# tangjiapeng/DiffuScene

Hardware: AMD Instinct MI355X
Metric: denoiser steps/sec (train + 1000-step sample) at B=256, N=80 objects (higher is better)
Workload: dtype f32 (operands split 3xbf16, 6 products, f32 accumulate); 1 GPU; uncond living/dining rooms (config/uncond/diffusion_livingrooms_instancond_lat32_v.yaml scaled to N=80), B=256 scenes per GPU, N=80, C=65, T=1000, mode=both; global_batch=256, parallelism=single

## Files before the change

__graft_entry__.py:

```python
import os
import subprocess
import sys

ROOT = os.path.dirname(os.path.abspath(__file__))
CSRC = os.path.join(ROOT, "diffuscene_amd", "csrc")
LIB = os.path.join(ROOT, "diffuscene_amd", "libdiffuscene_hip.so")

SOURCES = [
    ("gemm_mfma.hip", []),
    ("gemm_split.hip", ["-fno-slp-vectorize"]),
    ("gemm_tn_split.hip", ["-fno-slp-vectorize"]),
    ("blocks.hip", []),
    ("diffusion.hip", ["-ffp-contract=off"]),
    ("train.hip", []),
    ("retrieval.hip", ["-ffp-contract=off"]),
    ("dataset.hip", ["-ffp-contract=off"]),
    ("chamfer.hip", ["-ffp-contract=off"]),
    ("optim.hip", ["-ffp-contract=off"]),
    ("foldingnet.hip", []),
]


def _hipcc():
    for c in (os.environ.get("HIPCC"), "/opt/rocm/bin/hipcc", "hipcc"):
        if c and (os.path.isabs(c) and os.path.exists(c) or not os.path.isabs(c)):
            return c
    raise RuntimeError("hipcc not found")


def _stale(target, deps):
    if not os.path.exists(target):
        return True
    t = os.path.getmtime(target)
    return any(os.path.getmtime(d) > t for d in deps)


def _stamp_git_head():
    try:
        head = subprocess.check_output(["git", "rev-parse", "--short", "HEAD"], cwd=ROOT, stderr=subprocess.DEVNULL, text=True).strip()
        dirty = subprocess.check_output(["git", "status", "--porcelain", "-uno"], cwd=ROOT, stderr=subprocess.DEVNULL, text=True).strip()
        with open(os.path.join(ROOT, "GIT_HEAD"), "w") as f:
            f.write(head + ("+" if dirty else "") + "\n")
    except Exception:
        pass


def build(force=False):
    hipcc = _hipcc()
    headers = [os.path.join(CSRC, "dsc_common.h"), os.path.join(CSRC, "gemm_core.h"), os.path.join(CSRC, "gemm_tn_split.h"),
               os.path.join(ROOT, "include", "diffuscene_hip.h")]
    objs = []
    for src, extra in SOURCES:
        s = os.path.join(CSRC, src)
        if not os.path.exists(s):
            continue
        o = os.path.join(CSRC, src.replace(".hip", ".o"))
        if force or _stale(o, [s] + headers):
            cmd = [hipcc, "--offload-arch=gfx950", "-O3", "-std=c++17", "-fPIC", "-c", s, "-o", o] + extra
            subprocess.check_call(cmd)
        objs.append(o)
    if force or _stale(LIB, objs):
        subprocess.check_call([hipcc, "--offload-arch=gfx950", "-shared", "-fPIC", "-o", LIB] + objs)
    gsrc = os.path.join(ROOT, "tools", "guard_alloc.cpp")
    gso = os.path.join(ROOT, "tools", "_build", "libdsc_guard_alloc.so")
    if os.path.exists(gsrc) and (force or _stale(gso, [gsrc])):
        os.makedirs(os.path.dirname(gso), exist_ok=True)
        try:
            subprocess.check_call([hipcc, "-O2", "-std=c++17", "-fPIC", "-shared", gsrc, "-o", gso])
        except (subprocess.CalledProcessError, OSError) as e:
            print("warning: guard allocator (tools/guard_alloc.cpp) not built: %s -- tests/test_gpu_guard.py will skip its allocator runs" % e,
                  file=sys.stderr)
    _stamp_git_head()
    if ROOT not in sys.path:
        sys.path.insert(0, ROOT)
    import diffuscene_amd
    from diffuscene_amd import _lib
    _lib.load()
    import oracle.ref_torch


def build_asan():
    hipcc = _hipcc()
    out = os.path.join(ROOT, "diffuscene_amd", "libdiffuscene_hip_asan.so")
    objs = []
    for src, extra in SOURCES:
        s = os.path.join(CSRC, src)
        o = os.path.join(CSRC, src.replace(".hip", ".asan.o"))
        subprocess.check_call([hipcc, "--offload-arch=gfx950", "-O1", "-g", "-std=c++17", "-fPIC", "-fsanitize=address", "-fno-gpu-sanitize",
                               "-shared-libsan", "-Wno-option-ignored", "-c", s, "-o", o] + extra)
        objs.append(o)
    subprocess.check_call([hipcc, "--offload-arch=gfx950", "-shared", "-fPIC", "-fsanitize=address", "-fno-gpu-sanitize", "-shared-libsan",
                           "-Wno-option-ignored", "-o", out] + objs)
    return out


def smoke():
    if ROOT not in sys.path:
        sys.path.insert(0, ROOT)
    import torch
    assert torch.cuda.is_available(), "smoke() needs a GPU"
    from diffuscene_amd.networks.denoise_net import Unet1D
    from diffuscene_amd.networks.diffusion_ddpm import DiffusionPoint
    from oracle import ref_torch as R
    from oracle import weights as W

    kw = dict(W.UNCOND_BEDROOM)
    B, N = 4, 12
    dev = torch.device("cuda:0")
    net = Unet1D(**kw)
    sd = W.synth_state_dict(kw)
    net.load_state_dict(sd)
    net.to(dev)
    cfg = dict(objectness_dim=0, class_dim=22, angle_dim=2, objfeat_dim=32)
    diff = DiffusionPoint(net, cfg, time_num=1000, model_mean_type="v")
    x = W.synth_scene_batch(B, N, 22, 32, 0)
    t = torch.tensor([3, 250, 600, 999], dtype=torch.int64)
    cond = W.synth_condition(B, N, 128, 0).contiguous()
    noise = W.synth_noise((B, N, 62), 7)
    with torch.no_grad():
        out = net(x.to(dev), t.to(dev), cond.to(dev), None).cpu()
        ref = R.unet1d_forward(sd, kw, x, t, cond, None)
        rel = float((out - ref).abs().max() / ref.abs().max())
        assert rel < 1e-4, "Unet1D forward mismatch vs oracle: %g" % rel
        tb = R.schedule_tables(1e-4, 0.02, 1000, "v")
        step = diff.diffusion.p_sample(diff._denoise, x.to(dev), t.to(dev), cond.to(dev), None,
                                       noise_fn=lambda size, dtype, device: noise.to(device), clip_denoised=True).cpu()
        ref_step = R.p_sample_step(tb, x, t, ref, noise, True, "v")
        rel2 = float((step - ref_step).abs().max() / ref_step.abs().max())
        assert rel2 < 1e-4, "p_sample mismatch vs oracle: %g" % rel2
    print("smoke ok: forward rel err %.3g, p_sample rel err %.3g" % (rel, rel2))


if __name__ == "__main__":
    if "--asan" in sys.argv:
        print("built", build_asan())
        sys.exit(0)
    build(force="--force" in sys.argv)
    if "--smoke" in sys.argv:
        smoke()
```

diffuscene_amd/_lib.py:

```python
import ctypes as C
import os

_HERE = os.path.dirname(os.path.abspath(__file__))
LIB_PATH = os.path.join(_HERE, "libdiffuscene_hip.so")
if os.environ.get("DSC_HIP_LIB"):
    LIB_PATH = os.path.abspath(os.environ["DSC_HIP_LIB"])

ACT_NONE, ACT_GELU, ACT_SILU, ACT_LEAKY01 = 0, 1, 2, 3
SS_NONE, SS_PER_TOKEN, SS_PER_SCENE, SS_PER_SLOT, SS_BY_INDEX = 0, 1, 2, 3, 4
MEAN_EPS, MEAN_X0, MEAN_V = 0, 1, 2
TILE_GN_80_W8, TILE_GN_80_W4, TILE_160x256, TILE_160x128_W4 = 1, 2, 5, 8
TILE_WAVE_GN, TILE_WAVE_DENSE, TILE_WAVE_GN_64 = 10, 11, 12
F32_TILE_160x256, F32_TILE_160x128, F32_TILE_128x128, F32_TILE_96x128, F32_TILE_64x64 = 0, 1, 2, 3, 4
DSC_PLANES_NONE = -100
GEMM_ROW_INVARIANT = 1
WS_MAX = 64
MAX_TOKENS_PER_SCENE = 160
STATS_MAX_OBJECTS, STATS_ONE_WAVE_MAX = 160, 32

_ERR = {-1: "DSC_EINVAL (bad shape / null pointer)", -2: "DSC_EALIGN (16-byte alignment required)",
        -3: "DSC_ERANGE (size outside kernel limits)"}

c_f32p = C.c_void_p
c_i64p = C.c_void_p


class GemmArgs(C.Structure):
    _fields_ = [
        ("a1", C.c_void_p), ("lda1", C.c_int64), ("k1", C.c_int32),
        ("a2", C.c_void_p), ("lda2", C.c_int64), ("k2", C.c_int32),
        ("w", C.c_void_p), ("ldw", C.c_int64),
        ("bias", C.c_void_p),
        ("residual", C.c_void_p), ("ldr", C.c_int64),
        ("y", C.c_void_p), ("ldy", C.c_int64),
        ("m", C.c_int32), ("n", C.c_int32),
        ("act_in", C.c_int32), ("act_out", C.c_int32),
        ("batch", C.c_int32),
        ("sa1", C.c_int64), ("sa2", C.c_int64), ("sw", C.c_int64), ("sbias", C.c_int64),
        ("sres", C.c_int64), ("sy", C.c_int64),
        ("gamma", C.c_void_p), ("beta", C.c_void_p), ("eps", C.c_float),
        ("tokens_per_scene", C.c_int32),
        ("scale_shift", C.c_void_p), ("ld_ss", C.c_int64), ("ss_mode", C.c_int32),
        ("preact", C.c_void_p), ("ld_preact", C.c_int64),
        ("ss_index", C.c_void_p),
        ("w_planes", C.c_void_p),
        ("actgrad_x", C.c_void_p), ("ld_actgrad", C.c_int64),
        ("ss_rows", C.c_int32),
        ("w_planes_layout", C.c_int32),
        ("gnb_z", C.c_void_p), ("ld_gnb_z", C.c_int64),
        ("gnb_dgamma", C.c_void_p), ("gnb_dbeta", C.c_void_p), ("gnb_dbias", C.c_void_p), ("gnb_pstride", C.c_int64),
        ("gnb_dss", C.c_void_p), ("ld_gnb_dss", C.c_int64),
        ("flags", C.c_int32),
    ]


class SplitItem(C.Structure):
    _fields_ = [("w", C.c_void_p), ("ldw", C.c_int64), ("rows", C.c_int32), ("cols", C.c_int32), ("planes", C.c_void_p),
                ("transpose", C.c_int32)]


class SmallKItem(C.Structure):
    _fields_ = [("x", C.c_void_p), ("ldx", C.c_int64), ("k_in", C.c_int32), ("w", C.c_void_p), ("ldw", C.c_int64), ("bias", C.c_void_p),
                ("y", C.c_void_p), ("ldy", C.c_int64)]


class ColSpan(C.Structure):
    _fields_ = [("src_col", C.c_int32), ("dst_col", C.c_int32), ("width", C.c_int32)]


SMALLK_MAX = 4


class WsItem(C.Structure):
    _fields_ = [("w", C.c_void_p), ("out", C.c_void_p), ("rows", C.c_int32), ("cols", C.c_int32)]


class TnGroup(C.Structure):
    _fields_ = [("a1", C.c_void_p), ("lda1", C.c_int64), ("k1", C.c_int32),
                ("a2", C.c_void_p), ("lda2", C.c_int64), ("k2", C.c_int32),
                ("dy", C.c_void_p), ("ldd", C.c_int64),
                ("out", C.c_void_p), ("ldo", C.c_int64),
                ("dbias", C.c_void_p),
                ("m", C.c_int32), ("n", C.c_int32), ("kvalid", C.c_int32),
                ("tile0", C.c_int32),
                ("ws_offset", C.c_int64),
                ("tile0s", C.c_int32)]


class ColsumItem(C.Structure):
    _fields_ = [("x", C.c_void_p), ("ldx", C.c_int64), ("m", C.c_int32), ("n", C.c_int32), ("out", C.c_void_p)]


class WsBwdItem(C.Structure):
    _fields_ = [("w", C.c_void_p), ("dw_std", C.c_void_p), ("dw", C.c_void_p), ("rows", C.c_int32), ("cols", C.c_int32)]


SIGNATURES = {
    "dsc_version": (C.c_int, []),
    "dsc_gemm_f32": (C.c_int, [C.POINTER(GemmArgs), C.c_void_p]),
    "dsc_gemm_gn_silu_f32": (C.c_int, [C.POINTER(GemmArgs), C.c_void_p]),
    "dsc_split_bf16x3_f32": (C.c_int, [C.POINTER(SplitItem), C.c_int32, C.c_void_p]),
    "dsc_gemm_arithmetic": (C.c_int, [C.POINTER(GemmArgs), C.c_int32]),
    "dsc_gemm_split_tile": (C.c_int, [C.POINTER(GemmArgs), C.c_int32]),
    "dsc_gemm_f32_tile": (C.c_int, [C.POINTER(GemmArgs)]),
    "dsc_gemm_planes_layout": (C.c_int, [C.POINTER(GemmArgs), C.c_int32]),
    "dsc_get_split_wave": (C.c_int, []),
    "dsc_set_split_wave": (C.c_int, [C.c_int32]),
    "dsc_gemm_skinny": (C.c_int, [C.POINTER(GemmArgs), C.c_int32]),
    "dsc_get_skinny": (C.c_int, []),
    "dsc_set_skinny": (C.c_int, [C.c_int32]),
    "dsc_get_gemm_arithmetic": (C.c_int, []),
    "dsc_set_gemm_arithmetic": (C.c_int, [C.c_int32]),
    "dsc_gemm_layernorm_f32": (C.c_int, [C.POINTER(GemmArgs), C.c_void_p]),
    "dsc_gemm_splitk_f32": (C.c_int, [C.POINTER(GemmArgs), C.c_int32, c_f32p, C.c_int64, C.c_void_p]),
    "dsc_linear_smallk_f32": (C.c_int, [c_f32p, C.c_int64, C.c_int32, c_f32p, C.c_int64, c_f32p, c_f32p, C.c_int64,
                                        C.c_int32, C.c_int32, C.c_int32, C.c_void_p]),
    "dsc_linear_smallk_grouped_f32": (C.c_int, [C.POINTER(SmallKItem), C.c_int32, C.c_int32, C.c_int32, C.c_int32, C.c_void_p]),
    "dsc_gather_columns_f32": (C.c_int, [c_f32p, C.c_int64, c_f32p, C.c_int64, C.c_int32, C.POINTER(ColSpan), C.c_int32, C.c_void_p]),
    "dsc_weight_standardize_f32": (C.c_int, [C.POINTER(WsItem), C.c_int32, C.c_float, C.c_void_p]),
    "dsc_layernorm_f32": (C.c_int, [c_f32p, C.c_int64, c_f32p, c_f32p, C.c_int64, c_f32p, C.c_int64, C.c_int32,
                                    C.c_int32, C.c_float, C.c_void_p]),
    "dsc_linear_attention_f32": (C.c_int, [c_f32p, C.c_int64, c_f32p, C.c_int64, c_f32p, C.c_int64, c_f32p, C.c_int64,
                                           C.c_int32, C.c_int32, C.c_int32, C.c_float, C.c_void_p]),
    "dsc_attention_f32": (C.c_int, [c_f32p, C.c_int64, c_f32p, C.c_int64, c_f32p, C.c_int64, c_f32p, C.c_int64,
                                    C.c_int32, C.c_int32, C.c_float, C.c_void_p]),
    "dsc_time_embedding_f32": (C.c_int, [c_i64p, C.c_int32, C.c_int32, c_f32p, C.c_int32, c_f32p, c_f32p, C.c_void_p]),
    "dsc_activation_f32": (C.c_int, [c_f32p, c_f32p, C.c_int64, C.c_int32, C.c_void_p]),
    "dsc_q_sample_f32": (C.c_int, [c_f32p, c_f32p, c_i64p, c_f32p, c_f32p, c_f32p, c_f32p, C.c_int32, C.c_int64, C.c_int32,
                                   C.c_void_p]),
    "dsc_p_sample_f32": (C.c_int, [c_f32p, c_f32p, c_f32p, c_i64p, c_f32p, c_f32p, c_f32p, c_f32p, c_f32p, c_f32p,
                                   c_f32p, C.c_int32, C.c_int32, C.c_int32, C.c_int64, C.c_int32, C.c_void_p]),
    "dsc_device_error_count": (C.c_int64, [C.c_int32]),
    "dsc_add_scalar_i64": (C.c_int, [c_i64p, C.c_int32, C.c_int64, C.c_void_p]),
    "dsc_ddim_step_f32": (C.c_int, [c_f32p, c_f32p, c_f32p, c_i64p, c_i64p, c_i64p, c_f32p, c_f32p, c_f32p, c_f32p, c_f32p,
                                    c_f32p, c_f32p, c_f32p, c_f32p, C.c_int32, C.c_int32, C.c_int64, C.c_int32, C.c_int32,
                                    C.c_void_p]),
    "dsc_ddim_advance_i64": (C.c_int, [c_i64p, c_i64p, c_i64p, C.c_int32, C.c_int32, C.c_void_p]),
    "dsc_knn16_f32": (C.c_int, [c_f32p, C.c_int64, C.c_int32, c_f32p, c_f32p, C.c_int32, C.c_int32, C.c_void_p, C.c_void_p]),
    "dsc_rowsq_f32": (C.c_int, [c_f32p, C.c_int64, C.c_int32, C.c_int64, c_f32p, C.c_void_p]),
    "dsc_knn_cov_f32": (C.c_int, [c_f32p, C.c_int64, C.c_void_p, C.c_int32, C.c_int32, c_f32p, C.c_int64, C.c_void_p]),
    "dsc_gather_max_f32": (C.c_int, [c_f32p, C.c_int64, C.c_void_p, C.c_int32, C.c_int32, C.c_int32, c_f32p, C.c_int64,
                                     C.c_void_p, C.c_void_p]),
    "dsc_gather_max_bwd_f32": (C.c_int, [c_f32p, C.c_int64, C.c_void_p, C.c_void_p, C.c_int32, C.c_int32, C.c_int32, c_f32p,
                                         C.c_int64, C.c_void_p]),
    "dsc_bn_workspace_floats": (C.c_int64, [C.c_int64, C.c_int32]),
    "dsc_batchnorm_fwd_f32": (C.c_int, [c_f32p, C.c_int64, c_f32p, c_f32p, C.c_int64, C.c_int32, C.c_float, C.c_float,
                                        C.c_int32, c_f32p, c_f32p, c_f32p, c_f32p, c_f32p, c_f32p, c_f32p, C.c_int64,
                                        C.c_void_p]),
    "dsc_batchnorm_eval_f32": (C.c_int, [c_f32p, C.c_int64, c_f32p, c_f32p, c_f32p, c_f32p, C.c_int64, C.c_int32, C.c_int32,
                                         c_f32p, C.c_void_p]),
    "dsc_batchnorm_bwd_f32": (C.c_int, [c_f32p, c_f32p, c_f32p, c_f32p, c_f32p, C.c_int64, C.c_int32, C.c_int32, c_f32p,
                                        c_f32p, c_f32p, c_f32p, C.c_int64, C.c_void_p]),
    "dsc_rowmax_f32": (C.c_int, [c_f32p, C.c_int64, C.c_int32, C.c_int32, C.c_int32, c_f32p, C.c_void_p, C.c_void_p]),
    "dsc_rowmax_bwd_f32": (C.c_int, [c_f32p, C.c_void_p, C.c_int32, C.c_int32, C.c_int32, c_f32p, C.c_void_p]),
    "dsc_point_affine_f32": (C.c_int, [c_f32p, C.c_int64, C.c_int32, c_f32p, C.c_int64, c_f32p, C.c_int32, C.c_int32,
                                       C.c_int32, C.c_int32, c_f32p, C.c_void_p]),
    "dsc_point_affine_bwd_f32": (C.c_int, [c_f32p, c_f32p, C.c_int64, C.c_int32, c_f32p, C.c_int64, C.c_int32, C.c_int32,
                                           C.c_int32, C.c_int32, c_f32p, C.c_int64, c_f32p, C.c_int64, c_f32p, c_f32p,
                                           C.c_int64, C.c_void_p]),
    "dsc_postfilter_compact_f32": (C.c_int, [c_f32p, C.c_int32, C.c_int32, C.c_int32, C.c_int32, C.c_int32, C.c_int32, c_f32p,
                                             C.c_void_p, C.c_void_p]),
    "dsc_gemm_tn_f32": (C.c_int, [c_f32p, C.c_int64, C.c_int32, c_f32p, C.c_int64, C.c_int32, c_f32p, C.c_int64, c_f32p,
                                  C.c_int64, c_f32p, C.c_int32, C.c_int32, C.c_int32, c_f32p, C.c_int64, C.c_void_p]),
    "dsc_gemm_tn_workspace_floats": (C.c_int64, [C.c_int32, C.c_int32, C.c_int32]),
    "dsc_gemm_tn_grouped_f32": (C.c_int, [C.c_void_p, C.c_int32, C.c_int32, C.c_int32, c_f32p, C.c_int64, C.c_int64,
                                          C.c_void_p]),
    "dsc_gemm_tn_grouped_split_f32": (C.c_int, [C.c_void_p, C.c_int32, C.c_int32, C.c_void_p, C.c_int32, C.c_int32, c_f32p, C.c_int64,
                                                C.c_int64, C.c_int32, C.c_void_p]),
    "dsc_set_tn_split_form": (C.c_int, [C.c_int32]),
    "dsc_get_tn_split_form": (C.c_int, []),
    "dsc_colsum_f32": (C.c_int, [c_f32p, C.c_int64, C.c_int32, C.c_int32, c_f32p, c_f32p, C.c_int64, C.c_void_p]),
    "dsc_colsum_grouped_f32": (C.c_int, [C.c_void_p, C.c_int32, C.c_int32, C.c_void_p]),
    "dsc_gn_silu_bwd_f32": (C.c_int, [c_f32p, C.c_int64, c_f32p, C.c_int64, c_f32p, c_f32p, c_f32p, C.c_int64, C.c_int32,
                                      c_f32p, C.c_int64, c_f32p, c_f32p, c_f32p, C.c_int64, c_f32p, C.c_int64, C.c_int32,
                                      C.c_int32, C.c_int32, C.c_float, C.c_void_p]),
    "dsc_weight_standardize_bwd_f32": (C.c_int, [C.POINTER(WsBwdItem), C.c_int32, C.c_float, C.c_void_p]),
    "dsc_layernorm_bwd_f32": (C.c_int, [c_f32p, C.c_int64, c_f32p, c_f32p, C.c_int64, c_f32p, C.c_int64, c_f32p, C.c_int64, c_f32p,
                                        C.c_int32, C.c_int32, C.c_int32, C.c_float, C.c_void_p]),
    "dsc_linear_attention_bwd_f32": (C.c_int, [c_f32p, C.c_int64] * 7 + [C.c_int32, C.c_int32, C.c_int32, C.c_float,
                                                                          C.c_void_p]),
    "dsc_attention_bwd_f32": (C.c_int, [c_f32p, C.c_int64] * 7 + [C.c_int32, C.c_int32, C.c_float, C.c_void_p]),
    "dsc_retrieve_nearest_f32": (C.c_int, [c_f32p, C.c_void_p, C.c_void_p, c_f32p, C.c_void_p, C.c_void_p, C.c_int32,
                                           C.c_int32, C.c_int32, C.c_void_p, c_f32p, C.c_void_p]),
    "dsc_box_bounds_f32": (C.c_int, [c_f32p, c_f32p, c_f32p, C.c_void_p, C.c_int32, C.c_int32, c_f32p, C.c_void_p]),
    "dsc_scene_stats_f32": (C.c_int, [c_f32p, c_f32p, C.c_void_p, C.c_void_p, C.c_int32, C.c_int32, C.c_int32, C.c_int32,
                                      C.c_void_p, C.c_void_p, C.c_void_p, C.c_void_p, C.c_void_p, C.c_void_p, c_f32p, C.c_void_p]),
    "dsc_encode_scene_batch_f32": (C.c_int, [c_i64p, c_f32p, c_f32p, c_f32p, c_f32p, c_f32p, C.c_int32, C.c_int32, c_i64p,
                                             C.c_void_p, C.c_void_p, C.c_void_p, C.c_int32, C.POINTER(C.c_double), c_f32p,
                                             C.c_int64, c_i64p, C.c_int32, C.c_int32, C.c_void_p]),
    "dsc_chamfer3d_forward_f32": (C.c_int, [c_f32p, c_f32p, c_f32p, c_f32p, C.c_void_p, C.c_void_p, C.c_int32, C.c_int32,
                                            C.c_int32, C.c_void_p]),
    "dsc_chamfer3d_backward_f32": (C.c_int, [c_f32p, c_f32p, c_f32p, c_f32p, C.c_void_p, C.c_void_p, c_f32p, c_f32p,
                                             C.c_int32, C.c_int32, C.c_int32, C.c_void_p]),
    "dsc_grad_sumsq_f32": (C.c_int, [C.c_void_p, C.c_int32, C.c_void_p, C.c_void_p]),
    "dsc_clip_coef_f32": (C.c_int, [C.c_void_p, C.c_int32, C.c_float, c_f32p, c_f32p, C.c_void_p]),
    "dsc_adam_step_f32": (C.c_int, [C.c_void_p, C.c_int32, C.c_float, C.c_float, C.c_float, C.c_float, C.c_float, C.c_float,
                                    c_f32p, C.c_void_p]),
    "dsc_ddpm_loss_f32": (C.c_int, [c_f32p, c_f32p, c_f32p, c_i64p, c_f32p, c_f32p, c_f32p, c_f32p, C.POINTER(C.c_float),
                                    c_f32p, c_f32p, c_f32p] + [C.c_int32] * 12 + [C.c_float, C.c_int32, C.c_void_p]),
    "dsc_copy2d_f32": (C.c_int, [c_f32p, C.c_int64, c_f32p, C.c_int64, C.c_int32, C.c_int32, C.c_void_p]),
    "dsc_add2d_f32": (C.c_int, [c_f32p, C.c_int64, c_f32p, C.c_int64, C.c_int32, C.c_int32, C.c_void_p]),
    "dsc_activation_bwd_f32": (C.c_int, [c_f32p, c_f32p, c_f32p, C.c_int64, C.c_int32, C.c_void_p]),
    "dsc_transpose_batched_f32": (C.c_int, [C.POINTER(WsItem), C.c_int32, C.c_void_p]),
    "dsc_transpose_f32": (C.c_int, [c_f32p, C.c_int64, c_f32p, C.c_int64, C.c_int32, C.c_int32, C.c_void_p]),
    "dsc_complete_overwrite_f32": (C.c_int, [c_f32p, c_f32p, c_f32p, c_i64p, c_f32p, c_f32p, C.c_int32, C.c_int32,
                                             C.c_int32, C.c_int32, C.c_int32, C.c_void_p]),
    "dsc_complete_overwrite_ragged_f32": (C.c_int, [c_f32p, c_f32p, c_f32p, c_i64p, c_i64p, c_f32p, c_f32p, C.c_int32, C.c_int32,
                                                    C.c_int32, C.c_int32, C.c_int32, C.c_void_p]),
    "dsc_p_sample_inpaint_f32": (C.c_int, [c_f32p, c_f32p, c_f32p, c_f32p, c_f32p, c_i64p, c_i64p, c_f32p, c_f32p, c_f32p, c_f32p,
                                           c_f32p, c_f32p, c_f32p, c_f32p] + [C.c_int32] * 7 + [C.c_void_p]),
    "dsc_ddim_inpaint_step_f32": (C.c_int, [c_f32p] * 5 + [c_i64p] * 4 + [c_f32p] * 10 + [C.c_int32] * 7 + [C.c_void_p]),
    "dsc_masked_overwrite_f32": (C.c_int, [c_f32p, c_f32p, c_f32p, C.c_void_p, c_i64p, c_f32p, c_f32p, C.c_int32, C.c_int64, C.c_int32,
                                           C.c_void_p]),
    "dsc_p_sample_masked_f32": (C.c_int, [c_f32p] * 5 + [C.c_void_p, c_i64p] + [c_f32p] * 8 + [C.c_int32] * 3 + [C.c_int64, C.c_int32,
                                                                                                                  C.c_void_p]),
    "dsc_ddim_masked_step_f32": (C.c_int, [c_f32p] * 5 + [C.c_void_p] + [c_i64p] * 3 + [c_f32p] * 10 + [C.c_int32] * 2 +
                                 [C.c_int64, C.c_int32, C.c_int32, C.c_void_p]),
    "dsc_cfg_combine_f32": (C.c_int, [c_f32p, c_f32p, c_f32p, C.c_int32, C.c_int64, C.c_void_p]),
    "dsc_scene_randn_f32": (C.c_int, [c_f32p, c_i64p, c_i64p, C.c_int64, C.c_int64, C.c_int64, C.c_void_p]),
    "dsc_scene_philox_u32": (C.c_int, [C.c_void_p, c_i64p, c_i64p, C.c_int64, C.c_int64, C.c_int64, C.c_void_p]),
    "dsc_p_sample_cfg_f32": (C.c_int, [c_f32p] * 4 + [c_i64p] + [c_f32p] * 8 + [C.c_int32] * 3 + [C.c_int64, C.c_int32, C.c_void_p]),
    "dsc_ddim_cfg_step_f32": (C.c_int, [c_f32p] * 4 + [c_i64p] * 3 + [c_f32p] * 10 + [C.c_int32] * 2 +
                              [C.c_int64, C.c_int32, C.c_int32, C.c_void_p]),
    "dsc_scene_gate_f32": (C.c_int, [c_f32p, C.c_void_p, c_f32p, C.c_int32, C.c_int64, C.c_void_p]),
}

_lib = None


class HipLibraryMissing(RuntimeError):
    pass


def load():
    global _lib
    if _lib is not None:
        return _lib
    if not os.path.exists(LIB_PATH):
        raise HipLibraryMissing(
            "%s not found: build it with `python __graft_entry__.py` (hipcc --offload-arch=gfx950). "
            "diffuscene_amd has no CPU or PyTorch fallback." % LIB_PATH)
    import torch
    lib = C.CDLL(LIB_PATH)
    for name, (res, args) in SIGNATURES.items():
        try:
            fn = getattr(lib, name)
        except AttributeError as e:
            raise HipLibraryMissing("symbol %s missing from %s" % (name, LIB_PATH)) from e
        fn.restype = res
        fn.argtypes = args
    if lib.dsc_get_gemm_arithmetic() < 0:
        raise ValueError("DSC_GEMM=%r: must be 'split' (default) or 'f32'" % os.environ.get("DSC_GEMM"))
    if lib.dsc_get_tn_split_form() < 0:
        raise ValueError("DSC_TN_FORM=%r: must be '2' (default), '1' or '0'" % os.environ.get("DSC_TN_FORM"))
    if lib.dsc_get_split_wave() < 0:
        raise ValueError("DSC_WAVE=%r: must be '1' / 'auto' (default) or '0'" % os.environ.get("DSC_WAVE"))
    _lib = lib
    return lib


def split_enabled():
    return load().dsc_get_gemm_arithmetic() == 1


def gemm_mode():
    lib = load()
    if lib.dsc_get_gemm_arithmetic() != 1:
        return 0
    return (2 if lib.dsc_get_split_wave() == 1 else 1) + 10 * lib.dsc_get_tn_split_form()


def set_split_wave(on):
    prev = load().dsc_get_split_wave() == 1
    check(load().dsc_set_split_wave(1 if on else 0), "dsc_set_split_wave")
    return prev


def set_gemm_arithmetic(name):
    if name not in ("split", "f32"):
        raise ValueError("gemm arithmetic must be 'split' or 'f32', got %r" % (name,))
    prev = "split" if split_enabled() else "f32"
    check(load().dsc_set_gemm_arithmetic(1 if name == "split" else 0), "dsc_set_gemm_arithmetic")
    return prev


def device_error_count(reset=False):
    n = load().dsc_device_error_count(1 if reset else 0)
    if n < 0:
        raise RuntimeError("dsc_device_error_count failed (HIP error)")
    return int(n)


def check_indices(where):
    if os.environ.get("DSC_CHECK_INDICES", "0") == "1":
        n = device_error_count(reset=True)
        if n:
            raise IndexError("%s: %d out-of-range device timestep(s) were clamped into the schedule tables" % (where, n))


def check(rc, what):
    if rc != 0:
        raise RuntimeError("%s failed: %s" % (what, _ERR.get(rc, "hipError_t %d" % rc)))


def fn(name):
    return getattr(load(), name)
```

diffuscene_amd/csrc/gemm_split.hip:

```cpp
#include "dsc_common.h"
#include "gemm_split_wave.h"
#include <atomic>
#include <cstring>

#ifndef DSC_SPLIT_DSPREAD
#define DSC_SPLIT_DSPREAD true
#endif

namespace dsc_split {

typedef unsigned u32x4 __attribute__((ext_vector_type(4)));
typedef __bf16 bf16x8 __attribute__((ext_vector_type(8)));
typedef __bf16 bf16x2 __attribute__((ext_vector_type(2)));

constexpr int BK = 32;

__device__ __forceinline__ unsigned cvt_pk_bf16(float a, float b) {
    f32x2 v = {a, b};
    return __builtin_bit_cast(unsigned, __builtin_convertvector(v, bf16x2));
}
__device__ __forceinline__ float bf_lo(unsigned p) { return __builtin_bit_cast(float, p << 16); }
__device__ __forceinline__ float bf_hi(unsigned p) { return __builtin_bit_cast(float, p & 0xffff0000u); }

__device__ __forceinline__ void split8(const f32x4 lo, const f32x4 hi, bf16x8& p1, bf16x8& p2, bf16x8& p3) {
    u32x4 a, b, c;
#pragma unroll
    for (int q = 0; q < 4; ++q) {
        const float x0 = q < 2 ? lo[2 * q] : hi[2 * q - 4], x1 = q < 2 ? lo[2 * q + 1] : hi[2 * q - 3];
        const unsigned u1 = cvt_pk_bf16(x0, x1);
        const float r0 = x0 - bf_lo(u1), r1 = x1 - bf_hi(u1);
        const unsigned u2 = cvt_pk_bf16(r0, r1);
        const float s0 = r0 - bf_lo(u2), s1 = r1 - bf_hi(u2);
        a[q] = u1;
        b[q] = u2;
        c[q] = cvt_pk_bf16(s0, s1);
    }
    p1 = __builtin_bit_cast(bf16x8, a);
    p2 = __builtin_bit_cast(bf16x8, b);
    p3 = __builtin_bit_cast(bf16x8, c);
}

struct SplitBatch { dsc_split_item it[DSC_WS_MAX]; };

__global__ __launch_bounds__(256) void split_planes_kernel(const SplitBatch bch) {
    dsc_split_item it = bch.it[blockIdx.y];
    const bool frag = (it.transpose & DSC_SPLIT_FRAGMENT) != 0;
    it.transpose &= DSC_SPLIT_TRANSPOSE;
    const int ro = it.transpose ? it.cols : it.rows, co = it.transpose ? it.rows : it.cols;
    const int oct = co / 8;
    const long items = (long)ro * oct;
    const long plane = (long)ro * co;
    for (long i = (long)blockIdx.x * blockDim.x + threadIdx.x; i < items; i += (long)gridDim.x * blockDim.x) {
        const long r = it.transpose ? i % ro : i / oct;
        const long o = it.transpose ? i / ro : i % oct;
        f32x4 lo, hi;
        if (it.transpose) {
#pragma unroll
            for (int e = 0; e < 4; ++e) {
                lo[e] = it.w[(o * 8 + e) * it.ldw + r];
                hi[e] = it.w[(o * 8 + 4 + e) * it.ldw + r];
            }
        } else {
            lo = *reinterpret_cast<const f32x4*>(it.w + r * it.ldw + o * 8);
            hi = *reinterpret_cast<const f32x4*>(it.w + r * it.ldw + o * 8 + 4);
        }
        bf16x8 a, b, c;
        split8(lo, hi, a, b, c);
        uint16_t* d = it.planes + (frag ? ((((r >> 4) * (co >> 5) + (o >> 2)) * 64 + (o & 3) * 16 + (r & 15)) * 8) : (r * co + o * 8));
        *reinterpret_cast<bf16x8*>(d) = a;
        *reinterpret_cast<bf16x8*>(d + plane) = b;
        *reinterpret_cast<bf16x8*>(d + 2 * plane) = c;
    }
}

template <int WM, int WN, int RB>
constexpr int split_smem_bytes() {
    constexpr int BM = 16 * RB * WM, BN = 64 * WN;
    constexpr int STAGE = 3 * BM * BK * 2 + 3 * BN * BK * 2;
    constexpr int ITEMS_W = BM * 4 / (WM * WN);
    return 2 * STAGE + ((ITEMS_W % 64) ? 1024 : 0);
}

struct NoSync { __device__ __forceinline__ void operator()() const {} };

template <bool GN, int WM, int WN, int RB, bool DSPREAD, class Sync = NoSync>
__device__ __forceinline__ void gemm_split_tile(const dsc_gemm_args& p, const int ntok, const int bid, const int zb, char* const smem,
                                                const Sync sync = Sync{}) {
    constexpr int NW = WM * WN, T = 64 * NW;
    static_assert(NW == 8 || NW == 4, "4 or 8 waves");
    constexpr int BM = 16 * RB * WM, BN = 64 * WN;
    constexpr int B_PLANE = BN * BK * 2, X_PLANE = BM * BK * 2;
    constexpr int XA = 3 * X_PLANE, STAGE = XA + 3 * B_PLANE;
    constexpr int CH_PL = B_PLANE / 1024, CH = 3 * CH_PL, NI = (CH + NW - 1) / NW;
    constexpr int ITEMS_W = BM * 4 / NW;
    constexpr int NIT = (ITEMS_W + 63) / 64;
    constexpr int DUMP = (ITEMS_W % 64) ? 1024 : 0;
    static_assert(NIT <= RB && NIT <= 3, "the splits ride in the last NIT token blocks of a tile");
    static_assert(2 * STAGE + DUMP <= 160 * 1024, "two stages must fit the 160 KiB LDS");
    static_assert(2 * STAGE + DUMP == split_smem_bytes<WM, WN, RB>(), "split_smem_bytes");
    const int tid = threadIdx.x, lane = tid & 63, wave = tid >> 6;
    const int wave_u = __builtin_amdgcn_readfirstlane(wave);
    const int wm = wave_u % WM, wn = wave_u / WM;
    const int K = p.k1 + p.k2;
    const int scenes = (p.m + ntok - 1) / ntok;
    const int cbs = p.n / BN, rbs = (scenes + WM - 1) / WM;
    int rb, cb;
    if ((rbs & 7) == 0) {
        const int xcd = bid & 7, idx = bid >> 3;
        rb = xcd * (rbs >> 3) + idx / cbs;
        cb = idx % cbs;
    } else {
        rb = bid / cbs;
        cb = bid % cbs;
    }
    const int row0 = rb * WM * ntok, col0 = cb * BN;
    const int rows_here = p.m - row0;
    const int z = zb;
    const float* const xb1 = p.a1 + (int64_t)z * p.sa1 + (int64_t)row0 * p.lda1;
    const float* const xb2 = p.a2 ? p.a2 + (int64_t)z * p.sa2 + (int64_t)row0 * p.lda2 : xb1;
    const uint16_t* const wb = p.w_planes + ((int64_t)z * p.n + col0) * K;
    const int plane_bytes = p.batch * p.n * K * 2;
    const float* const bias = p.bias ? p.bias + (int64_t)z * p.sbias : nullptr;

    int dvoff[NI];
#pragma unroll
    for (int i = 0; i < NI; ++i) {
        int c = wave_u + NW * i;
        if (c >= CH) c -= CH;
        const int plane = c / CH_PL, nrow = (c % CH_PL) * 16 + (lane >> 2);
        dvoff[i] = plane * plane_bytes + nrow * K * 2 + (((lane & 3) ^ ((nrow >> 1) & 3)) << 4);
    }
    auto dma_part = [&](int kt, char* stage, auto i0c, auto i1c) {
        constexpr int i0 = decltype(i0c)::value, i1 = decltype(i1c)::value;
        __attribute__((address_space(3))) char* lbase = (__attribute__((address_space(3))) char*)stage;
#pragma unroll
        for (int i = i0; i < (i1 < NI ? i1 : NI); ++i) {
            int c = wave_u + NW * i;
            if (c >= CH) c -= CH;
#if defined(__HIP_DEVICE_COMPILE__)
            const __amdgpu_buffer_rsrc_t rs = __builtin_amdgcn_make_buffer_rsrc((void*)const_cast<uint16_t*>(wb), 0, 0x7fffffff, 0x00020000);
            __builtin_amdgcn_raw_ptr_buffer_load_lds(rs, lbase + XA + c * 1024, 16, dvoff[i], kt * BK * 2, 0, 0);
#else
            (void)lbase; (void)kt;
#endif
        }
    };
    auto dma_tile = [&](int kt, char* stage) { dma_part(kt, stage, std::integral_constant<int, 0>{}, std::integral_constant<int, NI>{}); };
    constexpr int PER = DSPREAD ? (NI + RB - 1) / RB : NI;

    f32x4 acc[RB][4];
    const int g = lane >> 4, l15 = lane & 15;
#pragma unroll
    for (int j = 0; j < 4; ++j) {
        f32x4 b4 = {0.f, 0.f, 0.f, 0.f};
        if (bias) b4 = *reinterpret_cast<const f32x4*>(bias + col0 + wn * 64 + j * 16 + 4 * g);
#pragma unroll
        for (int i = 0; i < RB; ++i) acc[i][j] = b4;
    }

    int woff[4];
#pragma unroll
    for (int j = 0; j < 4; ++j) {
        const int nr = wn * 64 + j * 16 + l15;
        woff[j] = XA + nr * 64 + ((g ^ ((nr >> 1) & 3)) << 4);
    }
    auto mma_block = [&](const bf16x8 (&wf)[4][3], const bf16x8& x1, const bf16x8& x2, const bf16x8& x3, f32x4 (&c)[4]) {
#pragma unroll
        for (int j = 0; j < 4; ++j) c[j] = __builtin_amdgcn_mfma_f32_16x16x32_bf16(wf[j][2], x1, c[j], 0, 0, 0);
#pragma unroll
        for (int j = 0; j < 4; ++j) c[j] = __builtin_amdgcn_mfma_f32_16x16x32_bf16(wf[j][0], x3, c[j], 0, 0, 0);
#pragma unroll
        for (int j = 0; j < 4; ++j) c[j] = __builtin_amdgcn_mfma_f32_16x16x32_bf16(wf[j][1], x2, c[j], 0, 0, 0);
#pragma unroll
        for (int j = 0; j < 4; ++j) c[j] = __builtin_amdgcn_mfma_f32_16x16x32_bf16(wf[j][1], x1, c[j], 0, 0, 0);
#pragma unroll
        for (int j = 0; j < 4; ++j) c[j] = __builtin_amdgcn_mfma_f32_16x16x32_bf16(wf[j][0], x2, c[j], 0, 0, 0);
#pragma unroll
        for (int j = 0; j < 4; ++j) c[j] = __builtin_amdgcn_mfma_f32_16x16x32_bf16(wf[j][0], x1, c[j], 0, 0, 0);
    };
    constexpr int NMMA = 24;

    int ioff1[NIT], ioff2[NIT], ildso[NIT];
    bool ion[NIT];
#pragma unroll
    for (int u = 0; u < NIT; ++u) {
        const int idx = 64 * u + lane;
        ion[u] = idx < ITEMS_W;
        const int t = wave_u * ITEMS_W + (ion[u] ? idx : 0);
        const int r = t >> 2, q = t & 3;
        const int sc = r / (16 * RB), tk = r % (16 * RB), gr = sc * ntok + tk;
        const int grow = (tk < ntok && gr < rows_here) ? gr : 0;
        ioff1[u] = grow * (int)p.lda1 * 4 + q * 32;
        ioff2[u] = grow * (int)p.lda2 * 4 + q * 32;
        ildso[u] = r * 64 + ((q ^ ((r >> 1) & 3)) << 4);
    }
    int xoff[RB];
#pragma unroll
    for (int i = 0; i < RB; ++i) {
        const int r = (wm * RB + i) * 16 + l15;
        xoff[i] = r * 64 + ((g ^ ((r >> 1) & 3)) << 4);
    }
    f32x4 ld[NIT][2];
    auto load_items = [&](int kt) {
        const int k0 = kt * BK;
        const bool seg1 = k0 < p.k1;
        const char* base = reinterpret_cast<const char*>(seg1 ? xb1 : xb2) + (seg1 ? k0 : k0 - p.k1) * 4;
#pragma unroll
        for (int u = 0; u < NIT; ++u) {
            const int o = seg1 ? ioff1[u] : ioff2[u];
            ld[u][0] = *reinterpret_cast<const f32x4*>(base + o);
            ld[u][1] = *reinterpret_cast<const f32x4*>(base + o + 16);
        }
    };
    auto store_item = [&](int u, char* stage) {
        bf16x8 a, b, c;
        split8(ld[u][0], ld[u][1], a, b, c);
        char* d0 = ion[u] ? stage + ildso[u] : smem + 2 * STAGE + lane * 16;
        const int ps = ion[u] ? X_PLANE : 0;
        *reinterpret_cast<bf16x8*>(d0) = a;
        *reinterpret_cast<bf16x8*>(d0 + ps) = b;
        *reinterpret_cast<bf16x8*>(d0 + 2 * ps) = c;
    };

    const int KT = K / BK;
    dma_tile(0, smem);
    sync();
    load_items(0);
#pragma unroll
    for (int u = 0; u < NIT; ++u) store_item(u, smem);
    for (int kt = 0; kt < KT; ++kt) {
        __builtin_amdgcn_s_waitcnt(0x0070);
        __syncthreads();
        char* cur = smem + (kt & 1) * STAGE;
        char* nxt = smem + ((kt + 1) & 1) * STAGE;
        const int kn = min(kt + 1, KT - 1);
        if constexpr (!DSPREAD) dma_tile(kn, nxt);
        load_items(kn);
        bf16x8 wf[4][3], xf[2][3];
#pragma unroll
        for (int pl = 0; pl < 3; ++pl) xf[0][pl] = *reinterpret_cast<const bf16x8*>(cur + pl * X_PLANE + xoff[0]);
#pragma unroll
        for (int j = 0; j < 4; ++j)
#pragma unroll
            for (int pl = 0; pl < 3; ++pl) wf[j][pl] = *reinterpret_cast<const bf16x8*>(cur + woff[j] + pl * B_PLANE);
        __builtin_amdgcn_sched_barrier(0);
#pragma unroll
        for (int i = 0; i < RB; ++i) {
            if (i + 1 < RB) {
#pragma unroll
                for (int pl = 0; pl < 3; ++pl) xf[(i + 1) & 1][pl] = *reinterpret_cast<const bf16x8*>(cur + pl * X_PLANE + xoff[i + 1]);
            }
            if (i == RB - NIT) {
                constexpr int FLY = DSPREAD ? (NI < RB * PER ? NI : RB * PER) : 0;
                __builtin_amdgcn_sched_barrier(0);
                __builtin_amdgcn_s_waitcnt(0x0f70 | (FLY & 15) | ((FLY >> 4) << 14));
                __builtin_amdgcn_sched_barrier(0);
            }
            if (i >= RB - NIT) store_item(i - (RB - NIT), nxt);
            if constexpr (DSPREAD) {
                if (i * PER < NI) {
                    if (i == 0) dma_part(kn, nxt, std::integral_constant<int, 0>{}, std::integral_constant<int, PER>{});
                    if (i == 1) dma_part(kn, nxt, std::integral_constant<int, PER>{}, std::integral_constant<int, 2 * PER>{});
                    if (i == 2) dma_part(kn, nxt, std::integral_constant<int, 2 * PER>{}, std::integral_constant<int, 3 * PER>{});
                    if (i == 3) dma_part(kn, nxt, std::integral_constant<int, 3 * PER>{}, std::integral_constant<int, 4 * PER>{});
                    if (i == 4) dma_part(kn, nxt, std::integral_constant<int, 4 * PER>{}, std::integral_constant<int, 5 * PER>{});
                }
            }
            mma_block(wf, xf[i & 1][0], xf[i & 1][1], xf[i & 1][2], acc[i]);
            __builtin_amdgcn_sched_group_barrier(0x008, 1, 0);
            if (i + 1 < RB) __builtin_amdgcn_sched_group_barrier(0x100, 3, 0);
            if constexpr (DSPREAD) {
                if (i * PER < NI) {
#pragma unroll
                    for (int q = 0; q < PER; ++q) {
                        __builtin_amdgcn_sched_group_barrier(0x008, 2, 0);
                        __builtin_amdgcn_sched_group_barrier(0x020, 1, 0);
                    }
                }
            }
            if (i >= RB - NIT) {
#pragma unroll
                for (int q = 0; q < NMMA - 2; ++q) {
                    __builtin_amdgcn_sched_group_barrier(0x008, 1, 0);
                    __builtin_amdgcn_sched_group_barrier(0x002, (44 + NMMA - 3) / (NMMA - 2), 0);
                }
                __builtin_amdgcn_sched_group_barrier(0x008, 1, 0);
                __builtin_amdgcn_sched_group_barrier(0x200, 3, 0);
            }
            __builtin_amdgcn_sched_barrier(0);
        }
    }
    __builtin_amdgcn_s_waitcnt(0x0f70);

    const int cbase = col0 + wn * 64 + 4 * g;
    const int srow = wm * ntok;
    bool valid[RB];
#pragma unroll
    for (int i = 0; i < RB; ++i) valid[i] = i * 16 + l15 < ntok && srow + i * 16 + l15 < rows_here;
    float* const ob = p.y + (int64_t)z * p.sy + (int64_t)(row0 + srow + l15) * p.ldy + cbase;
    const float* const rbp = p.residual ? p.residual + (int64_t)z * p.sres + (int64_t)(row0 + srow + l15) * p.ldr + cbase : nullptr;
    if constexpr (!GN) {
        float* const ub = p.preact ? p.preact + (int64_t)z * p.sy + (int64_t)(row0 + srow + l15) * p.ld_preact + cbase : nullptr;
        const float* const gb = p.actgrad_x ? p.actgrad_x + (int64_t)z * p.sy + (int64_t)(row0 + srow + l15) * p.ld_actgrad + cbase : nullptr;
#pragma unroll
        for (int i = 0; i < RB; ++i) {
            if (valid[i]) {
#pragma unroll
                for (int j = 0; j < 4; ++j) {
                    f32x4 y = acc[i][j];
                    if (ub) *reinterpret_cast<f32x4*>(ub + (int64_t)i * 16 * p.ld_preact + j * 16) = y;
                    if (gb) {
                        const f32x4 u = *reinterpret_cast<const f32x4*>(gb + (int64_t)i * 16 * p.ld_actgrad + j * 16);
#pragma unroll
                        for (int e = 0; e < 4; ++e) y[e] *= dsc_act_grad(u[e], p.act_out);
                    } else if (p.act_out != DSC_ACT_NONE) {
#pragma unroll
                        for (int e = 0; e < 4; ++e) y[e] = dsc_act(y[e], p.act_out);
                    }
                    if (rbp) y += *reinterpret_cast<const f32x4*>(rbp + (int64_t)i * 16 * p.ldr + j * 16);
                    *reinterpret_cast<f32x4*>(ob + (int64_t)i * 16 * p.ldy + j * 16) = y;
                }
            }
        }
    } else {
        const int scene = min(row0 / ntok + wm, p.m / ntok - 1);
        const bool per_row = p.ss_mode == DSC_SS_PER_TOKEN || p.ss_mode == DSC_SS_PER_SLOT;
        f32x4 ga[4], be[4], sc[4], sh[4];
        int64_t ssrow = scene;
        if (p.ss_mode == DSC_SS_BY_INDEX) ssrow = dsc_clamp_index(p.ss_index[scene], p.ss_rows);
#pragma unroll
        for (int j = 0; j < 4; ++j) {
            ga[j] = *reinterpret_cast<const f32x4*>(p.gamma + cbase + j * 16);
            be[j] = *reinterpret_cast<const f32x4*>(p.beta + cbase + j * 16);
            if (p.ss_mode == DSC_SS_PER_SCENE || p.ss_mode == DSC_SS_BY_INDEX) {
                const float* ssr = p.scale_shift + ssrow * p.ld_ss + cbase + j * 16;
                sc[j] = *reinterpret_cast<const f32x4*>(ssr);
                sh[j] = *reinterpret_cast<const f32x4*>(ssr + p.n);
            } else {
                sc[j] = f32x4{0.f, 0.f, 0.f, 0.f};
                sh[j] = sc[j];
            }
        }
        if (p.preact) {
            float* const pb = p.preact + (int64_t)(row0 + srow + l15) * p.ld_preact + cbase;
#pragma unroll
            for (int i = 0; i < RB; ++i)
                if (valid[i]) {
#pragma unroll
                    for (int j = 0; j < 4; ++j) *reinterpret_cast<f32x4*>(pb + (int64_t)i * 16 * p.ld_preact + j * 16) = acc[i][j];
                }
        }
        const float inv_cnt = 1.f / (float)(ntok * 64);
        float s0 = 0.f;
#pragma unroll
        for (int i = 0; i < RB; ++i)
#pragma unroll
            for (int j = 0; j < 4; ++j)
                s0 += valid[i] ? (acc[i][j][0] + acc[i][j][1]) + (acc[i][j][2] + acc[i][j][3]) : 0.f;
        const float mean = wave_sum_dpp(s0) * inv_cnt;
        float q0 = 0.f;
#pragma unroll
        for (int i = 0; i < RB; ++i)
#pragma unroll
            for (int j = 0; j < 4; ++j)
#pragma unroll
                for (int e = 0; e < 4; ++e) {
                    const float d = valid[i] ? acc[i][j][e] - mean : 0.f;
                    q0 = fmaf(d, d, q0);
                }
        const float rstd = 1.f / sqrtf(wave_sum_dpp(q0) * inv_cnt + p.eps);
#pragma unroll
        for (int j = 0; j < 4; ++j)
#pragma unroll
            for (int e = 0; e < 4; ++e) {
                const float a = rstd * ga[j][e], sp1 = sc[j][e] + 1.f;
                ga[j][e] = a * sp1;
                be[j][e] = fmaf(be[j][e] - mean * a, sp1, sh[j][e]);
            }
#pragma unroll
        for (int i = 0; i < RB; ++i) {
            if (valid[i]) {
#pragma unroll
                for (int j = 0; j < 4; ++j) {
                    f32x4 y, s1 = {1.f, 1.f, 1.f, 1.f}, s2 = {0.f, 0.f, 0.f, 0.f};
                    if (per_row) {
                        const int64_t row = p.ss_mode == DSC_SS_PER_TOKEN ? (int64_t)row0 + srow + i * 16 + l15 : (int64_t)i * 16 + l15;
                        const float* ssr = p.scale_shift + row * p.ld_ss + cbase + j * 16;
                        s1 = *reinterpret_cast<const f32x4*>(ssr) + 1.f;
                        s2 = *reinterpret_cast<const f32x4*>(ssr + p.n);
                    }
#pragma unroll
                    for (int e = 0; e < 4; ++e) {
                        float t = fmaf(acc[i][j][e], ga[j][e], be[j][e]);
                        if (per_row) t = fmaf(t, s1[e], s2[e]);
                        y[e] = dsc_silu_fast(t);
                    }
                    if (rbp) y += *reinterpret_cast<const f32x4*>(rbp + (int64_t)i * 16 * p.ldr + j * 16);
                    *reinterpret_cast<f32x4*>(ob + (int64_t)i * 16 * p.ldy + j * 16) = y;
                }
            }
        }
    }
}

template <bool GN, int WM, int WN, int RB, bool DSPREAD = DSC_SPLIT_DSPREAD>
__global__ __launch_bounds__(64 * WM * WN, 1) void gemm_split_kernel(const dsc_gemm_args p, const int ntok) {
    __shared__ __attribute__((aligned(16))) char smem[split_smem_bytes<WM, WN, RB>()];
    gemm_split_tile<GN, WM, WN, RB, DSPREAD>(p, ntok, blockIdx.x, blockIdx.y, smem);
}

template <bool GN, int WM, int WN, int RB>
int launch(const dsc_gemm_args* a, int ntok, hipStream_t s) {
    constexpr int BN = 64 * WN;
    const int scenes = (a->m + ntok - 1) / ntok;
    const unsigned grid = (unsigned)(((scenes + WM - 1) / WM) * (a->n / BN));
    DSC_CLEAR_STALE_ERROR();
    hipLaunchKernelGGL((gemm_split_kernel<GN, WM, WN, RB>), dim3(grid, (unsigned)a->batch), dim3(64 * WM * WN), 0, s, *a, ntok);
    DSC_LAUNCH_CHECK();
    return 0;
}

}

enum { T_GN_32 = 0, T_GN_80_W8, T_GN_80_W4, T_GN_48, T_GN_64, T_160x256, T_256x128, T_128x128, T_160x128_W4, T_64x256, T_WAVE_GN, T_WAVE_DENSE, T_WAVE_GN_64 };

static std::atomic<int> g_gemm_arith{-1000};

extern "C" int dsc_get_gemm_arithmetic(void) {
    int m = g_gemm_arith.load(std::memory_order_relaxed);
    if (m == -1000) {
        const char* e = getenv("DSC_GEMM");
        m = (!e || !e[0] || !strcmp(e, "split")) ? 1 : !strcmp(e, "f32") ? 0 : DSC_EINVAL;
        g_gemm_arith.store(m, std::memory_order_relaxed);
    }
    return m;
}

extern "C" int dsc_set_gemm_arithmetic(int32_t mode) {
    if (mode != 0 && mode != 1) return DSC_EINVAL;
    g_gemm_arith.store(mode, std::memory_order_relaxed);
    return 0;
}

static std::atomic<int> g_split_wave{-1000};

extern "C" int dsc_get_split_wave(void) {
    int m = g_split_wave.load(std::memory_order_relaxed);
    if (m == -1000) {
        const char* e = getenv("DSC_WAVE");
        m = (!e || !e[0] || !strcmp(e, "1") || !strcmp(e, "auto")) ? 1 : !strcmp(e, "0") ? 0 : DSC_EINVAL;
        g_split_wave.store(m, std::memory_order_relaxed);
    }
    return m;
}

extern "C" int dsc_set_split_wave(int32_t mode) {
    if (mode != 0 && mode != 1) return DSC_EINVAL;
    g_split_wave.store(mode, std::memory_order_relaxed);
    return 0;
}

static int select_wave(const dsc_gemm_args* a, bool gn) {
    if (dsc_get_split_wave() != 1) return -1;
    const int K = a->k1 + a->k2;
    if ((a->n % 128) || (a->k1 % 64) || (a->k2 % 64) || K < 256) return -1;
    if (a->batch != 1 && (gn || a->sw != (int64_t)a->n * K || a->ldw != K || (a->sy & 3) || (a->sres & 3) || (a->sbias & 3))) return -1;
    if (!dsc_aligned16(a->y) || (a->ldy & 3) || a->ldy < a->n) return -1;
    if (a->bias && !dsc_aligned16(a->bias)) return -1;
    if (a->residual && (!dsc_aligned16(a->residual) || (a->ldr & 3) || a->ldr < a->n)) return -1;
    if (a->preact && (!dsc_aligned16(a->preact) || (a->ld_preact & 3) || a->ld_preact < a->n || a->batch != 1)) return -1;
    if (a->actgrad_x && (gn || !dsc_aligned16(a->actgrad_x) || (a->ld_actgrad & 3) || a->ld_actgrad < a->n || a->batch != 1)) return -1;
    if (3LL * a->batch * a->n * K * 2 >= 0x7fffffffLL) return -1;
    const int64_t ld_max = a->lda1 > a->lda2 ? a->lda1 : a->lda2;
    if (ld_max * 4 * 96 >= 0x7fffffffLL) return -1;
    long waves;
    if (a->gnb_z) {
        const int N = a->tokens_per_scene;
        if (gn || a->batch != 1 || N <= 64 || N > 80 || (a->m % N) || a->bias || a->residual || a->preact || a->actgrad_x || a->act_out != DSC_ACT_NONE) return -1;
        if (!a->gamma || !a->beta || !a->gnb_dgamma || !a->gnb_dbeta || !a->gnb_dbias || (a->ss_mode != DSC_SS_NONE && a->ss_mode != DSC_SS_PER_SCENE)) return -1;
        if (!dsc_aligned16(a->gnb_z) || (a->ld_gnb_z & 3) || a->ld_gnb_z < a->n || !dsc_aligned16(a->gamma) || !dsc_aligned16(a->beta)) return -1;
        if (!dsc_aligned16(a->gnb_dgamma) || !dsc_aligned16(a->gnb_dbeta) || !dsc_aligned16(a->gnb_dbias) || (a->gnb_pstride & 3)) return -1;
        if (a->ss_mode == DSC_SS_PER_SCENE && (!a->scale_shift || !dsc_aligned16(a->scale_shift) || (a->ld_ss & 3))) return -1;
        if (a->gnb_dss && (!dsc_aligned16(a->gnb_dss) || (a->ld_gnb_dss & 3))) return -1;
        waves = (long)(a->m / N) * (a->n / 128);
        const long r = (waves + 1023) / 1024;
        return waves * 5 >= r * 1024 * 4 ? T_WAVE_DENSE : -1;
    }
    if (gn) {
        const int N = a->tokens_per_scene;
        if (N <= 16 || N > 80) return -1;
        const bool perrow = a->ss_mode == DSC_SS_PER_TOKEN || a->ss_mode == DSC_SS_PER_SLOT;
        if (perrow && a->ld_ss < 2 * (int64_t)a->n) return -1;
        waves = (long)(a->m / N) * (a->n / 128);
    } else {
        waves = (long)((a->m + 79) / 80) * (a->n / 128) * a->batch;
    }
    const long rounds = (waves + 1023) / 1024;
    if (waves * 5 >= rounds * 1024 * 4) return gn ? T_WAVE_GN : T_WAVE_DENSE;
    if (gn && a->tokens_per_scene > 64) {
        const long w4 = 2 * waves, r4 = (w4 + 1023) / 1024;
        if (r4 == 1 && w4 * 5 >= 1024 * 4) return T_WAVE_GN_64;
    }
    return -1;
}

static int select_block_tile(const dsc_gemm_args* a, bool gn);

static int select_tile(const dsc_gemm_args* a, bool gn, bool assume_planes = false) {
    if (dsc_get_gemm_arithmetic() != 1 || (!assume_planes && !a->w_planes)) return -1;
    if (a->flags & DSC_GEMM_ROW_INVARIANT) return -1;
    const int w = select_wave(a, gn);
    return w >= 0 ? w : select_block_tile(a, gn);
}

static int select_block_tile(const dsc_gemm_args* a, bool gn) {
    if (a->gnb_z) return -1;
    const int K = a->k1 + a->k2;
    if (a->batch != 1 && (gn || a->sw != (int64_t)a->n * K || a->ldw != K || (a->sy & 3) || (a->sres & 3) || (a->sbias & 3))) return -1;
    if ((a->n % 128) || (K % 32)) return -1;
    if (!dsc_aligned16(a->w_planes) || !dsc_aligned16(a->y) || (a->ldy & 3)) return -1;
    if (a->bias && !dsc_aligned16(a->bias)) return -1;
    if (a->residual && (!dsc_aligned16(a->residual) || (a->ldr & 3))) return -1;
    if (!gn && a->preact && (!dsc_aligned16(a->preact) || (a->ld_preact & 3) || a->batch != 1)) return -1;
    if (a->actgrad_x && (gn || !dsc_aligned16(a->actgrad_x) || (a->ld_actgrad & 3) || a->batch != 1)) return -1;
    if (3LL * a->batch * a->n * K * 2 >= 0x7fffffffLL) return -1;
    const int64_t ld_max = a->lda1 > a->lda2 ? a->lda1 : a->lda2;
    if (ld_max * 4 * 320 >= 0x7fffffffLL) return -1;
    const bool wide = (a->n % 256) == 0;
    constexpr long MIN_BLOCKS = 160;
    if (gn) {
        const int N = a->tokens_per_scene;
        if (N <= 16 || N > 80) return -1;
        const long S = a->m / N;
        if (N <= 32) return ((S + 3) / 4) * (a->n / 128) >= MIN_BLOCKS ? T_GN_32 : -1;
        const long b8 = wide ? ((S + 1) / 2) * (a->n / 256) : 0, b4 = ((S + 1) / 2) * (a->n / 128);
        if (N > 64) return b8 >= MIN_BLOCKS + 32 ? T_GN_80_W8 : b4 >= MIN_BLOCKS ? T_GN_80_W4 : -1;
        if (b8 < MIN_BLOCKS) return -1;
        return N <= 48 ? T_GN_48 : T_GN_64;
    }
    struct Cand { int bm, bn, id; };
    const Cand cands[5] = {{160, 256, T_160x256}, {256, 128, T_256x128}, {160, 128, T_160x128_W4}, {128, 128, T_128x128}, {64, 256, T_64x256}};
    int best = -1;
    long best_cost = 0, best_blk = 0;
    for (int i = 0; i < 5; ++i) {
        if (cands[i].bn == 256 && !wide) continue;
        const long nblk = (long)((a->m + cands[i].bm - 1) / cands[i].bm) * (a->n / cands[i].bn) * a->batch;
        const long c = ((nblk + 255) / 256) * (long)cands[i].bm * cands[i].bn;
        if (best < 0 || c < best_cost) { best = cands[i].id; best_cost = c; best_blk = nblk; }
    }
    return best_blk >= MIN_BLOCKS ? best : -1;
}

int dsc_gemm_try_split(const dsc_gemm_args* a, bool gn, hipStream_t s) {
    using namespace dsc_split;
    if (dsc_get_gemm_arithmetic() < 0 || dsc_get_split_wave() < 0) return DSC_EINVAL;
    const int N = a->tokens_per_scene;
    const int tile = select_tile(a, gn);
    if (tile < 0) return DSC_SPLIT_NOT_TAKEN;
    const int want = (tile == T_WAVE_GN || tile == T_WAVE_DENSE || tile == T_WAVE_GN_64) ? DSC_PLANES_FRAGMENT : DSC_PLANES_ROWMAJOR;
    if (a->w_planes_layout != want) return DSC_EINVAL;
    switch (tile) {
        case T_GN_32: return launch<true, 4, 2, 2>(a, N, s);
        case T_GN_80_W8: return launch<true, 2, 4, 5>(a, N, s);
        case T_GN_80_W4: return launch<true, 2, 2, 5>(a, N, s);
        case T_GN_48: return launch<true, 2, 4, 3>(a, N, s);
        case T_GN_64: return launch<true, 2, 4, 4>(a, N, s);
        case T_160x256: return launch<false, 2, 4, 5>(a, 80, s);
        case T_256x128: return launch<false, 4, 2, 4>(a, 64, s);
        case T_128x128: return launch<false, 4, 2, 2>(a, 32, s);
        case T_160x128_W4: return launch<false, 2, 2, 5>(a, 80, s);
        case T_64x256: return launch<false, 2, 4, 2>(a, 32, s);
        case T_WAVE_DENSE:
            if (a->gnb_z) return dsc_wave::launch<false, 5, false, 8, true>(a, a->w_planes, N, s);
            return dsc_wave::launch<false, 5>(a, a->w_planes, 80, s);
        case T_WAVE_GN_64:
            return (a->ss_mode == DSC_SS_PER_TOKEN || a->ss_mode == DSC_SS_PER_SLOT) ? dsc_wave::launch<true, 5, true, 4>(a, a->w_planes, N, s)
                                                                                     : dsc_wave::launch<true, 5, false, 4>(a, a->w_planes, N, s);
        case T_WAVE_GN: {
            const bool perrow = a->ss_mode == DSC_SS_PER_TOKEN || a->ss_mode == DSC_SS_PER_SLOT;
            const int rb = (N + 15) / 16;
            if (perrow) {
                return rb == 5 ? dsc_wave::launch<true, 5, true>(a, a->w_planes, N, s) : rb == 4 ? dsc_wave::launch<true, 4, true>(a, a->w_planes, N, s)
                     : rb == 3 ? dsc_wave::launch<true, 3, true>(a, a->w_planes, N, s) : dsc_wave::launch<true, 2, true>(a, a->w_planes, N, s);
            }
            return rb == 5 ? dsc_wave::launch<true, 5>(a, a->w_planes, N, s) : rb == 4 ? dsc_wave::launch<true, 4>(a, a->w_planes, N, s)
                 : rb == 3 ? dsc_wave::launch<true, 3>(a, a->w_planes, N, s) : dsc_wave::launch<true, 2>(a, a->w_planes, N, s);
        }
        default: return DSC_SPLIT_NOT_TAKEN;
    }
}

extern "C" int dsc_gemm_arithmetic(const dsc_gemm_args* a, int32_t gn) {
    if (!a || a->m <= 0 || a->n <= 0 || a->k1 <= 0) return DSC_EINVAL;
    return select_tile(a, gn != 0) >= 0 ? 1 : 0;
}

extern "C" int dsc_gemm_split_tile(const dsc_gemm_args* a, int32_t gn) {
    if (!a || a->m <= 0 || a->n <= 0 || a->k1 <= 0) return DSC_EINVAL;
    return select_tile(a, gn != 0);
}

extern "C" int dsc_gemm_planes_layout(const dsc_gemm_args* a, int32_t gn) {
    if (!a || a->m <= 0 || a->n <= 0 || a->k1 <= 0) return DSC_EINVAL;
    const int tile = select_tile(a, gn != 0, true);
    return tile < 0 ? DSC_PLANES_NONE : (tile == T_WAVE_GN || tile == T_WAVE_DENSE || tile == T_WAVE_GN_64) ? DSC_PLANES_FRAGMENT : DSC_PLANES_ROWMAJOR;
}

extern "C" int dsc_split_bf16x3_f32(const dsc_split_item* items, int32_t count, dsc_stream_t stream) {
    using namespace dsc_split;
    if (!items || count < 1 || count > DSC_WS_MAX) return DSC_EINVAL;
    SplitBatch b;
    long max_items = 0;
    for (int i = 0; i < count; ++i) {
        const dsc_split_item& it = items[i];
        if (!it.w || !it.planes || it.rows <= 0 || it.cols <= 0) return DSC_EINVAL;
        if (it.transpose & ~(DSC_SPLIT_TRANSPOSE | DSC_SPLIT_FRAGMENT)) return DSC_EINVAL;
        const bool tr = (it.transpose & DSC_SPLIT_TRANSPOSE) != 0;
        const int co = tr ? it.rows : it.cols, ro = tr ? it.cols : it.rows;
        if (co % 8) return DSC_EINVAL;
        if ((it.transpose & DSC_SPLIT_FRAGMENT) && ((ro % 16) || (co % 32))) return DSC_EINVAL;
        if (!dsc_aligned16(it.planes) || (!tr && (!dsc_aligned16(it.w) || (it.ldw & 3)))) return DSC_EALIGN;
        b.it[i] = it;
        const long n = (long)it.rows * it.cols / 8;
        if (n > max_items) max_items = n;
    }
    long bx = (max_items + 255) / 256;
    if (bx > 1024) bx = 1024;
    DSC_CLEAR_STALE_ERROR();
    hipLaunchKernelGGL(split_planes_kernel, dim3((unsigned)bx, (unsigned)count), dim3(256), 0, static_cast<hipStream_t>(stream), b);
    DSC_LAUNCH_CHECK();
    return 0;
}
```

diffuscene_amd/csrc/gemm_split_wave.h:

```cpp
#pragma once
#include "dsc_common.h"
#include <utility>

#ifndef DSC_WAVE_STAMP_ARGS
#define DSC_WAVE_STAMP_ARGS
#define DSC_WAVE_STAMP_PASS
#define DSC_WAVE_STAMP_DECL
#define DSC_WAVE_STAMP_KERNEL(id)
#define DSC_WAVE_STAMP_TILE(id)
#define DSC_WAVE_STAMP_FLUSH(kt)
#define DSC_WAVE_STAMP_END
#endif

namespace dsc_wave {

typedef unsigned u32x4 __attribute__((ext_vector_type(4)));
typedef __bf16 bf16x8 __attribute__((ext_vector_type(8)));
typedef __bf16 bf16x2 __attribute__((ext_vector_type(2)));

constexpr int BK = 32;
constexpr int WAVES = 4;

__device__ __forceinline__ unsigned cvt_pk_bf16(float a, float b) {
    f32x2 v = {a, b};
    return __builtin_bit_cast(unsigned, __builtin_convertvector(v, bf16x2));
}
__device__ __forceinline__ float bf_lo(unsigned p) { return __builtin_bit_cast(float, p << 16); }
__device__ __forceinline__ float bf_hi(unsigned p) { return __builtin_bit_cast(float, p & 0xffff0000u); }

__device__ __forceinline__ void split8(const f32x4 lo, const f32x4 hi, bf16x8& p1, bf16x8& p2, bf16x8& p3) {
    u32x4 a, b, c;
#pragma unroll
    for (int q = 0; q < 4; ++q) {
        const float x0 = q < 2 ? lo[2 * q] : hi[2 * q - 4], x1 = q < 2 ? lo[2 * q + 1] : hi[2 * q - 3];
        const unsigned u1 = cvt_pk_bf16(x0, x1);
        const float r0 = x0 - bf_lo(u1), r1 = x1 - bf_hi(u1);
        const unsigned u2 = cvt_pk_bf16(r0, r1);
        const float s0 = r0 - bf_lo(u2), s1 = r1 - bf_hi(u2);
        a[q] = u1;
        b[q] = u2;
        c[q] = cvt_pk_bf16(s0, s1);
    }
    p1 = __builtin_bit_cast(bf16x8, a);
    p2 = __builtin_bit_cast(bf16x8, b);
    p3 = __builtin_bit_cast(bf16x8, c);
}

template <int RB>
constexpr int wave_smem_bytes() { return WAVES * 2 * 3 * (16 * RB) * 64; }

template <bool GN, int RB, bool PERROW = false, int J = 8, bool GB = false>
__global__ __launch_bounds__(64 * WAVES, 1) void gemm_split_wave_kernel(const dsc_gemm_args p, const uint16_t* const planes_f, const int ntok DSC_WAVE_STAMP_ARGS) {
    static_assert(J == 8 || J == 4, "wave tile: 128 or 64 channels");
    static_assert(!GB || (!GN && J == 8), "the GroupNorm-backward epilogue rides on the dense 80 x 128 form");
    constexpr int NWF = 3 * J;
    constexpr int CW = 16 * J;
    constexpr int ROWS = 16 * RB, XP = ROWS * 64, STAGE = 3 * XP;
    constexpr int NWB = RB > 4 ? RB - 2 : RB > 3 ? RB - 1 : RB;
    constexpr int PERW = (NWF + NWB - 1) / NWB;
    __shared__ __attribute__((aligned(16))) char smem[wave_smem_bytes<RB>()];
    const int lane = threadIdx.x & 63;
    const int wave = __builtin_amdgcn_readfirstlane(threadIdx.x >> 6);
    const int K = p.k1 + p.k2, KT = K / BK;
    const int scenes = (p.m + ntok - 1) / ntok;
    const int sgs = (scenes + WAVES - 1) / WAVES, chunks = p.n / CW;
    const int bid = blockIdx.x;
    int sg, ch;
    if ((sgs & 7) == 0) {
        const int xcd = bid & 7, idx = bid >> 3;
        sg = xcd * (sgs >> 3) + idx / chunks;
        ch = idx % chunks;
    } else {
        sg = bid / chunks;
        ch = bid % chunks;
    }
    const int scene = sg * WAVES + wave;
    if (scene >= scenes) return;
    DSC_WAVE_STAMP_DECL
    DSC_WAVE_STAMP_KERNEL(0)
    const int z = blockIdx.y;
    const int row0 = scene * ntok, col0 = ch * CW;
    const int rows_here = min(ntok, p.m - row0);
    const float* const xb1 = p.a1 + (int64_t)z * p.sa1 + (int64_t)row0 * p.lda1;
    const float* const xb2 = p.a2 ? p.a2 + (int64_t)z * p.sa2 + (int64_t)row0 * p.lda2 : xb1;
    const float* const bias = p.bias ? p.bias + (int64_t)z * p.sbias : nullptr;
    const int64_t rec1 = ((int64_t)(p.m - row0 - 1) * p.lda1 + p.k1) * 4;
    const int64_t rec2 = p.a2 ? ((int64_t)(p.m - row0 - 1) * p.lda2 + p.k2) * 4 : rec1;
    const int64_t recw = (int64_t)3 * p.batch * p.n * K * 2;
    const int64_t rec1c = rec1 < 0x7fffffffLL ? rec1 : 0x7fffffffLL, rec2c = rec2 < 0x7fffffffLL ? rec2 : 0x7fffffffLL;
#if defined(__HIP_DEVICE_COMPILE__)
    const __amdgpu_buffer_rsrc_t r1 = __builtin_amdgcn_make_buffer_rsrc(const_cast<float*>(xb1), 0, (int)rec1c, 0x00020000);
    const __amdgpu_buffer_rsrc_t r2 = __builtin_amdgcn_make_buffer_rsrc(const_cast<float*>(xb2), 0, (int)rec2c, 0x00020000);
#endif
#if defined(__HIP_DEVICE_COMPILE__)
    const __amdgpu_buffer_rsrc_t rw = __builtin_amdgcn_make_buffer_rsrc(const_cast<uint16_t*>(planes_f), 0, (int)recw, 0x00020000);
#endif
    const int plane_bytes = p.batch * p.n * K * 2;
    const int nb0 = (z * p.n + col0) / 16;

    const int q4 = lane & 3, r16 = lane >> 2, g = lane >> 4, l15 = lane & 15;
    const int tvo1 = (r16 * (int)p.lda1 + q4 * 8) * 4, tvo2 = (r16 * (int)p.lda2 + q4 * 8) * 4;
    const int ildso = r16 * 64 + ((q4 ^ ((r16 >> 1) & 3)) << 4);
    const int xoff = l15 * 64 + ((g ^ ((l15 >> 1) & 3)) << 4);
    const int wvo = lane * 16;
    char* const wl = smem + wave * (2 * STAGE);

    f32x4 acc[RB][J];
#pragma unroll
    for (int j = 0; j < J; ++j) {
        f32x4 b4 = {0.f, 0.f, 0.f, 0.f};
        if (bias) b4 = *reinterpret_cast<const f32x4*>(bias + col0 + j * 16 + 4 * g);
#pragma unroll
        for (int i = 0; i < RB; ++i) acc[i][j] = b4;
    }

    f32x4 ld[RB][2];
    bf16x8 wf[2][J][3], xf[2][3];
    const int lda2e = p.a2 ? (int)p.lda2 : (int)p.lda1, kshift = p.a2 ? p.k1 : 0;
    const int tvo2e = p.a2 ? tvo2 : tvo1;
    auto load_tok = [&](int kt, int u, auto segc) {
#if defined(__HIP_DEVICE_COMPILE__)
        constexpr int SEG = decltype(segc)::value;
        const int k0 = kt * BK;
        if constexpr (SEG == 0) {
            const int so = (u * 16 * (int)p.lda1 + k0) * 4;
            ld[u][0] = __builtin_bit_cast(f32x4, __builtin_amdgcn_raw_buffer_load_b128(r1, tvo1, so, 0));
            ld[u][1] = __builtin_bit_cast(f32x4, __builtin_amdgcn_raw_buffer_load_b128(r1, tvo1 + 16, so, 0));
        } else {
            const int so = (u * 16 * lda2e + k0 - kshift) * 4;
            ld[u][0] = __builtin_bit_cast(f32x4, __builtin_amdgcn_raw_buffer_load_b128(r2, tvo2e, so, 0));
            ld[u][1] = __builtin_bit_cast(f32x4, __builtin_amdgcn_raw_buffer_load_b128(r2, tvo2e + 16, so, 0));
        }
#else
        (void)kt; (void)u;
#endif
    };
    auto load_w = [&](int kt, int j, int pl) -> bf16x8 {
#if defined(__HIP_DEVICE_COMPILE__)
        return __builtin_bit_cast(bf16x8, __builtin_amdgcn_raw_buffer_load_b128(rw, wvo, pl * plane_bytes + ((nb0 + j) * KT + kt) * 1024, 0));
#else
        (void)kt; (void)j; (void)pl;
        return bf16x8{};
#endif
    };
    constexpr int NMMA = 6 * J;

    auto tile = [&](const int kt, auto curc, auto segc) {
        constexpr int CUR = decltype(curc)::value, NXT = CUR ^ 1;
        char* const cur = wl + CUR * STAGE;
        char* const nxt = wl + NXT * STAGE;
        const int kn1 = min(kt + 1, KT - 1), kn2 = min(kt + 2, KT - 1);
        constexpr int X0 = CUR ? (RB & 1) : 0;
        DSC_WAVE_STAMP_TILE(0)
        auto block = [&](auto ic) {
            constexpr int i = decltype(ic)::value;
            constexpr int NR = 3;
            constexpr int W0 = i * PERW < NWF ? i * PERW : NWF, W1 = (i + 1) * PERW < NWF ? (i + 1) * PERW : NWF;
            constexpr int VPS = J == 8 ? 2 : 4, NVS = 44 / VPS;
            constexpr int S0 = NR + (W1 - W0), S1 = S0 + NVS, S2 = S1 + 3, S3 = S2 + 1;
            static_assert(S3 <= NMMA, "one MFMA per filler slot");
            unsigned su1[4], su2[4], su3[4];
            float sr0[4], sr1[4], st0[4], st1[4];
            auto xin = [&](int q, int h) -> float { return q < 2 ? ld[i][0][2 * q + h] : ld[i][1][2 * q - 4 + h]; };
            auto split_op = [&](auto nc) {
                constexpr int n = decltype(nc)::value;
                constexpr int q = 2 * (n / 22) + (n & 1), o = (n % 22) >> 1;
                if constexpr (o == 0) su1[q] = cvt_pk_bf16(xin(q, 0), xin(q, 1));
                if constexpr (o == 1) st0[q] = bf_lo(su1[q]);
                if constexpr (o == 2) st1[q] = bf_hi(su1[q]);
                if constexpr (o == 3) sr0[q] = xin(q, 0) - st0[q];
                if constexpr (o == 4) sr1[q] = xin(q, 1) - st1[q];
                if constexpr (o == 5) su2[q] = cvt_pk_bf16(sr0[q], sr1[q]);
                if constexpr (o == 6) st0[q] = bf_lo(su2[q]);
                if constexpr (o == 7) st1[q] = bf_hi(su2[q]);
                if constexpr (o == 8) sr0[q] = sr0[q] - st0[q];
                if constexpr (o == 9) sr1[q] = sr1[q] - st1[q];
                if constexpr (o == 10) su3[q] = cvt_pk_bf16(sr0[q], sr1[q]);
            };
            char* const d0 = nxt + i * 1024 + ildso;
            auto filler = [&](auto kc) {
                constexpr int k = decltype(kc)::value;
                if constexpr (k < NR) {
                    if constexpr (i + 1 < RB) xf[(X0 + i + 1) & 1][k] = *reinterpret_cast<const bf16x8*>(cur + k * XP + (i + 1) * 1024 + xoff);
                    else xf[(X0 + i + 1) & 1][k] = *reinterpret_cast<const bf16x8*>(nxt + k * XP + xoff);
                } else if constexpr (k < S0) {
                    constexpr int w = W0 + (k - NR);
                    wf[NXT][w / 3][w % 3] = load_w(kn1, w / 3, w % 3);
                } else if constexpr (k < S1) {
                    dsc_static_for<VPS>([&](auto vc) { split_op(std::integral_constant<int, VPS * (k - S0) + decltype(vc)::value>{}); });
                } else if constexpr (k < S2) {
                    constexpr int pl = k - S1;
                    const u32x4 v = pl == 0 ? u32x4{su1[0], su1[1], su1[2], su1[3]} : pl == 1 ? u32x4{su2[0], su2[1], su2[2], su2[3]}
                                                                                              : u32x4{su3[0], su3[1], su3[2], su3[3]};
                    *reinterpret_cast<u32x4*>(d0 + pl * XP) = v;
                } else if constexpr (k == S2) {
                    load_tok(kn2, i, segc);
                }
            };
            auto product = [&](auto pc) {
                constexpr int pr = decltype(pc)::value;
                constexpr int wp = pr == 0 ? 2 : (pr == 1 || pr >= 4) ? 0 : 1;
                constexpr int xp = pr == 0 ? 0 : pr == 1 ? 2 : pr == 2 ? 1 : pr == 3 ? 0 : pr == 4 ? 1 : 0;
                dsc_static_for<J>([&](auto jc) {
                    constexpr int j = decltype(jc)::value;
                    acc[i][j] = __builtin_amdgcn_mfma_f32_16x16x32_bf16(wf[CUR][j][wp], xf[(X0 + i) & 1][xp], acc[i][j], 0, 0, 0);
                    filler(std::integral_constant<int, pr * J + j>{});
                    __builtin_amdgcn_sched_barrier(0);
                });
            };
            dsc_static_for<6>(product);
            DSC_WAVE_STAMP_TILE(1 + i)
        };
        dsc_static_for<RB>(block);
        DSC_WAVE_STAMP_FLUSH(kt)
    };

    using std::integral_constant;
#pragma unroll
    for (int u = 0; u < RB; ++u) load_tok(0, u, integral_constant<int, 0>{});
#pragma unroll
    for (int w = 0; w < NWF; ++w) wf[0][w / 3][w % 3] = load_w(0, w / 3, w % 3);
#pragma unroll
    for (int u = 0; u < RB; ++u) {
        bf16x8 a, b, c;
        split8(ld[u][0], ld[u][1], a, b, c);
        char* d0 = wl + u * 1024 + ildso;
        *reinterpret_cast<bf16x8*>(d0) = a;
        *reinterpret_cast<bf16x8*>(d0 + XP) = b;
        *reinterpret_cast<bf16x8*>(d0 + 2 * XP) = c;
        load_tok(1, u, integral_constant<int, 0>{});
    }
#pragma unroll
    for (int pl = 0; pl < 3; ++pl) xf[0][pl] = *reinterpret_cast<const bf16x8*>(wl + pl * XP + xoff);
    const int KT1 = p.k1 / BK;
    int kt = 0;
    DSC_WAVE_STAMP_KERNEL(1)
    for (; kt + 2 < KT1; kt += 2) {
        tile(kt, integral_constant<int, 0>{}, integral_constant<int, 0>{});
        tile(kt + 1, integral_constant<int, 1>{}, integral_constant<int, 0>{});
    }
    f32x4 ep_ga[2], ep_be[2], ep_sc[2], ep_sh[2];
    if constexpr (GN) {
        const bool per_scene_e = p.ss_mode == DSC_SS_PER_SCENE || p.ss_mode == DSC_SS_BY_INDEX;
        int64_t ssrow_e = scene;
        if (p.ss_mode == DSC_SS_BY_INDEX) ssrow_e = dsc_clamp_index(p.ss_index[scene], p.ss_rows);
#pragma unroll
        for (int c2 = 0; c2 < J / 4; ++c2) {
            const int ch = col0 + 64 * c2 + 4 * (lane & 15);
            ep_ga[c2] = *reinterpret_cast<const f32x4*>(p.gamma + ch);
            ep_be[c2] = *reinterpret_cast<const f32x4*>(p.beta + ch);
            ep_sc[c2] = f32x4{0.f, 0.f, 0.f, 0.f};
            ep_sh[c2] = ep_sc[c2];
            if (per_scene_e) {
                const float* ssr = p.scale_shift + ssrow_e * p.ld_ss + ch;
                ep_sc[c2] = *reinterpret_cast<const f32x4*>(ssr);
                ep_sh[c2] = *reinterpret_cast<const f32x4*>(ssr + p.n);
            }
        }
    }
    for (; kt < KT; kt += 2) {
        tile(kt, integral_constant<int, 0>{}, integral_constant<int, 1>{});
        tile(kt + 1, integral_constant<int, 1>{}, integral_constant<int, 1>{});
    }

    DSC_WAVE_STAMP_KERNEL(2)
    constexpr int ERS = 64 * 4 + 16;
    static_assert(ROWS * ERS <= 2 * STAGE, "the transposed cell fits the wave's LDS image");
    const int er = lane >> 4, ec = lane & 15;
#if defined(__HIP_DEVICE_COMPILE__)
    auto row_rsrc = [&](const float* base, int64_t ld, int rows, int cols) {
        return __builtin_amdgcn_make_buffer_rsrc(const_cast<float*>(base), 0, rows > 0 ? (int)(((int64_t)(rows - 1) * ld + cols) * 4) : 0, 0x00020000);
    };
    const __amdgpu_buffer_rsrc_t ry = row_rsrc(p.y + (int64_t)z * p.sy + (int64_t)row0 * p.ldy, p.ldy, rows_here, p.n);
    const __amdgpu_buffer_rsrc_t rr = row_rsrc(p.residual ? p.residual + (int64_t)z * p.sres + (int64_t)row0 * p.ldr : p.y, p.ldr, p.residual ? rows_here : 0, p.n);
    const __amdgpu_buffer_rsrc_t rpa = row_rsrc(p.preact ? p.preact + (int64_t)z * p.sy + (int64_t)row0 * p.ld_preact : p.y, p.ld_preact, p.preact ? rows_here : 0, p.n);
    auto ld4 = [&](const __amdgpu_buffer_rsrc_t& r, int voff, int soff) { return __builtin_bit_cast(f32x4, __builtin_amdgcn_raw_buffer_load_b128(r, voff, soff, 0)); };
    auto st4 = [&](const f32x4 v, const __amdgpu_buffer_rsrc_t& r, int voff, int soff) { __builtin_amdgcn_raw_buffer_store_b128(__builtin_bit_cast(u32x4, v), r, voff, soff, 0); };
#else
    const int ry = 0, rr = 0, rpa = 0;
    auto ld4 = [&](int, int, int) { return f32x4{}; };
    auto st4 = [&](const f32x4, int, int, int) {};
#endif
    const bool has_res = p.residual != nullptr, has_pre = p.preact != nullptr;
    auto to_lds = [&](const int c2) {
#pragma unroll
        for (int i = 0; i < RB; ++i)
#pragma unroll
            for (int j = 0; j < 4; ++j) *reinterpret_cast<f32x4*>(wl + (i * 16 + l15) * ERS + (j * 16 + 4 * g) * 4) = acc[i][4 * c2 + j];
    };
    constexpr int NQ = ROWS / 4, QH = NQ % 10 == 0 ? 10 : NQ % 8 == 0 ? 8 : NQ % 6 == 0 ? 6 : 4;
    static_assert(NQ % QH == 0, "row groups per pass");
    if constexpr (GB) {
        const float inv_cnt = 1.f / (float)(ntok * 64);
        const bool per_scene = p.ss_mode == DSC_SS_PER_SCENE && p.scale_shift;
#if defined(__HIP_DEVICE_COMPILE__)
        const __amdgpu_buffer_rsrc_t rz = row_rsrc(p.gnb_z + (int64_t)row0 * p.ld_gnb_z, p.ld_gnb_z, rows_here, p.n);
#else
        const int rz = 0;
#endif
        dsc_static_for<2>([&](auto c2c) {
            constexpr int c2 = decltype(c2c)::value;
            const int ch = col0 + 64 * c2 + 4 * ec, cc = ch * 4;
            const int vy = er * (int)p.ldy * 4 + cc, vz = er * (int)p.ld_gnb_z * 4 + cc;
            f32x4 zv[NQ], dv[NQ];
#pragma unroll
            for (int q = 0; q < NQ; ++q) zv[q] = ld4(rz, vz, 4 * q * (int)p.ld_gnb_z * 4);
            const f32x4 ga = *reinterpret_cast<const f32x4*>(p.gamma + ch), be = *reinterpret_cast<const f32x4*>(p.beta + ch);
            f32x4 s1 = {1.f, 1.f, 1.f, 1.f}, sh = {0.f, 0.f, 0.f, 0.f};
            if (per_scene) {
                const float* ssr = p.scale_shift + (int64_t)scene * p.ld_ss + ch;
                s1 = *reinterpret_cast<const f32x4*>(ssr) + 1.f;
                sh = *reinterpret_cast<const f32x4*>(ssr + p.n);
            }
            to_lds(c2);
            float s = 0.f;
#pragma unroll
            for (int q = 0; q < NQ; ++q) {
                dv[q] = *reinterpret_cast<const f32x4*>(wl + (4 * q + er) * ERS + ec * 16);
                const bool ok = 4 * q + er < rows_here;
                if (!ok) dv[q] = f32x4{0.f, 0.f, 0.f, 0.f};
                s += ok ? (zv[q][0] + zv[q][1]) + (zv[q][2] + zv[q][3]) : 0.f;
            }
            const float mu = wave_sum_dpp(s) * inv_cnt;
            s = 0.f;
#pragma unroll
            for (int q = 0; q < NQ; ++q) {
                const bool ok = 4 * q + er < rows_here;
#pragma unroll
                for (int e = 0; e < 4; ++e) { const float d = ok ? zv[q][e] - mu : 0.f; s = fmaf(d, d, s); }
            }
            const float rs = 1.0f / sqrtf(wave_sum_dpp(s) * inv_cnt + p.eps);
            float S1 = 0.f, S2 = 0.f;
            f32x4 Gg = {0.f, 0.f, 0.f, 0.f}, Gb = Gg, Gsc = Gg, Gsh = Gg, Gz = Gg;
#pragma unroll
            for (int q = 0; q < NQ; ++q) {
#pragma unroll
                for (int e = 0; e < 4; ++e) {
                    const float xh = (zv[q][e] - mu) * rs;
                    const float gh = ga[e] * xh + be[e];
                    const float u = gh * s1[e] + sh[e];
                    const float sig = __builtin_amdgcn_rcpf(1.0f + __expf(-u));
                    const float du = dv[q][e] * (sig * (1.0f + u * (1.0f - sig)));
                    const float dgh = du * s1[e];
                    const float dxh = dgh * ga[e];
                    S1 += dxh; S2 += dxh * xh;
                    Gg[e] += dgh * xh; Gb[e] += dgh; Gsc[e] += du * gh; Gsh[e] += du;
                    zv[q][e] = xh;
                    dv[q][e] = dxh;
                }
            }
            const float m1 = wave_sum_dpp(S1) * inv_cnt, m2 = wave_sum_dpp(S2) * inv_cnt;
#pragma unroll
            for (int q = 0; q < NQ; ++q) {
                const bool ok = 4 * q + er < rows_here;
                f32x4 dzv;
#pragma unroll
                for (int e = 0; e < 4; ++e) { dzv[e] = rs * (dv[q][e] - m1 - zv[q][e] * m2); Gz[e] += ok ? dzv[e] : 0.f; }
                st4(dzv, ry, vy, 4 * q * (int)p.ldy * 4);
            }
            auto fold = [&](f32x4 v) {
#pragma unroll
                for (int e = 0; e < 4; ++e) { v[e] += __shfl_xor(v[e], 16, 64); v[e] += __shfl_xor(v[e], 32, 64); }
                return v;
            };
            Gg = fold(Gg); Gb = fold(Gb); Gz = fold(Gz);
            if (per_scene && p.gnb_dss) { Gsc = fold(Gsc); Gsh = fold(Gsh); }
            if (lane < 16) {
                const int64_t o = (int64_t)scene * p.gnb_pstride + ch;
                *reinterpret_cast<f32x4*>(p.gnb_dgamma + o) = Gg;
                *reinterpret_cast<f32x4*>(p.gnb_dbeta + o) = Gb;
                *reinterpret_cast<f32x4*>(p.gnb_dbias + o) = Gz;
                if (per_scene && p.gnb_dss) {
                    *reinterpret_cast<f32x4*>(p.gnb_dss + (int64_t)scene * p.ld_gnb_dss + ch) = Gsc;
                    *reinterpret_cast<f32x4*>(p.gnb_dss + (int64_t)scene * p.ld_gnb_dss + p.n + ch) = Gsh;
                }
            }
        });
    } else if constexpr (!GN) {
#if defined(__HIP_DEVICE_COMPILE__)
        const __amdgpu_buffer_rsrc_t rg = row_rsrc(p.actgrad_x ? p.actgrad_x + (int64_t)z * p.sy + (int64_t)row0 * p.ld_actgrad : p.y, p.ld_actgrad, p.actgrad_x ? rows_here : 0, p.n);
#else
        const int rg = 0;
#endif
        auto cell = [&](auto c2c, auto modec, auto actc) {
            constexpr int c2 = decltype(c2c)::value, MODE = decltype(modec)::value, ACT = decltype(actc)::value;
            const int cc = (col0 + 64 * c2 + 4 * ec) * 4;
            const int vy = er * (int)p.ldy * 4 + cc, vr = er * (int)p.ldr * 4 + cc, vp = er * (int)p.ld_preact * 4 + cc, vg = er * (int)p.ld_actgrad * 4 + cc;
            to_lds(c2);
#pragma unroll 1
            for (int h = 0; h < NQ; h += QH) {
                f32x4 rres[QH], gx[QH];
                if (has_res) {
#pragma unroll
                    for (int qq = 0; qq < QH; ++qq) rres[qq] = ld4(rr, vr, 4 * (h + qq) * (int)p.ldr * 4);
                }
                if constexpr (MODE == 2) {
#pragma unroll
                    for (int qq = 0; qq < QH; ++qq) gx[qq] = ld4(rg, vg, 4 * (h + qq) * (int)p.ld_actgrad * 4);
                }
#pragma unroll
                for (int qq = 0; qq < QH; ++qq) {
                    f32x4 y = *reinterpret_cast<const f32x4*>(wl + (4 * (h + qq) + er) * ERS + ec * 16);
                    if (has_pre) st4(y, rpa, vp, 4 * (h + qq) * (int)p.ld_preact * 4);
#pragma unroll
                    for (int e = 0; e < 4; ++e) {
                        if constexpr (MODE == 1) y[e] = dsc_act(y[e], ACT);
                        if constexpr (MODE == 2) y[e] *= dsc_act_grad(gx[qq][e], ACT);
                    }
                    if (has_res) y += rres[qq];
                    st4(y, ry, vy, 4 * (h + qq) * (int)p.ldy * 4);
                }
            }
        };
        auto cells = [&](auto modec, auto actc) {
            cell(std::integral_constant<int, 0>{}, modec, actc);
            if constexpr (J == 8) cell(std::integral_constant<int, 1>{}, modec, actc);
        };
        using std::integral_constant;
        const int act = p.act_out;
        if (p.actgrad_x) {
            if (act == DSC_ACT_GELU) cells(integral_constant<int, 2>{}, integral_constant<int, DSC_ACT_GELU>{});
            else if (act == DSC_ACT_SILU) cells(integral_constant<int, 2>{}, integral_constant<int, DSC_ACT_SILU>{});
            else if (act == DSC_ACT_LEAKY01) cells(integral_constant<int, 2>{}, integral_constant<int, DSC_ACT_LEAKY01>{});
            else cells(integral_constant<int, 0>{}, integral_constant<int, DSC_ACT_NONE>{});
        } else {
            if (act == DSC_ACT_GELU) cells(integral_constant<int, 1>{}, integral_constant<int, DSC_ACT_GELU>{});
            else if (act == DSC_ACT_SILU) cells(integral_constant<int, 1>{}, integral_constant<int, DSC_ACT_SILU>{});
            else if (act == DSC_ACT_LEAKY01) cells(integral_constant<int, 1>{}, integral_constant<int, DSC_ACT_LEAKY01>{});
            else cells(integral_constant<int, 0>{}, integral_constant<int, DSC_ACT_NONE>{});
        }
    } else {
#if defined(__HIP_DEVICE_COMPILE__)
        const __amdgpu_buffer_rsrc_t rs = row_rsrc(PERROW ? p.scale_shift + (p.ss_mode == DSC_SS_PER_TOKEN ? (int64_t)row0 * p.ld_ss : 0) : p.y, p.ld_ss,
                                                   PERROW ? rows_here : 0, 2 * p.n);
#else
        const int rs = 0;
#endif
        const float inv_cnt = 1.f / (float)(ntok * 64);
        const bool vlast = (RB - 1) * 16 + l15 < rows_here;
#pragma unroll
        for (int c2 = 0; c2 < J / 4; ++c2) {
            const int ch = col0 + 64 * c2 + 4 * ec;
            const f32x4 ga = ep_ga[c2], be = ep_be[c2], sc = ep_sc[c2], sh = ep_sh[c2];
            to_lds(c2);
            float s0 = 0.f;
#pragma unroll
            for (int i = 0; i < RB; ++i)
#pragma unroll
                for (int j = 0; j < 4; ++j) {
                    const f32x4 a = acc[i][4 * c2 + j];
                    const float t = (a[0] + a[1]) + (a[2] + a[3]);
                    s0 += (i < RB - 1 || vlast) ? t : 0.f;
                }
            const float mean = wave_sum_dpp(s0) * inv_cnt;
            float q0 = 0.f;
#pragma unroll
            for (int i = 0; i < RB; ++i)
#pragma unroll
                for (int j = 0; j < 4; ++j)
#pragma unroll
                    for (int e = 0; e < 4; ++e) {
                        const float d = (i < RB - 1 || vlast) ? acc[i][4 * c2 + j][e] - mean : 0.f;
                        q0 = fmaf(d, d, q0);
                    }
            const float rstd = 1.f / sqrtf(wave_sum_dpp(q0) * inv_cnt + p.eps);
            if (c2 == 0) { DSC_WAVE_STAMP_KERNEL(3) }
            f32x4 A, B;
#pragma unroll
            for (int e = 0; e < 4; ++e) {
                const float a = rstd * ga[e], sp1 = sc[e] + 1.f;
                A[e] = a * sp1;
                B[e] = fmaf(be[e] - mean * a, sp1, sh[e]);
            }
            const int cc = ch * 4;
            const int vy = er * (int)p.ldy * 4 + cc, vr = er * (int)p.ldr * 4 + cc, vp = er * (int)p.ld_preact * 4 + cc, vs = er * (int)p.ld_ss * 4 + cc;
            if (c2 == 0) { DSC_WAVE_STAMP_KERNEL(4) }
#pragma unroll
            for (int h = 0; h < NQ; h += QH) {
                f32x4 rres[QH], s1[QH], s2[QH];
                if (has_res) {
#pragma unroll
                    for (int qq = 0; qq < QH; ++qq) rres[qq] = ld4(rr, vr, 4 * (h + qq) * (int)p.ldr * 4);
                }
                if constexpr (PERROW) {
#pragma unroll
                    for (int qq = 0; qq < QH; ++qq) {
                        s1[qq] = ld4(rs, vs, 4 * (h + qq) * (int)p.ld_ss * 4);
                        s2[qq] = ld4(rs, vs + p.n * 4, 4 * (h + qq) * (int)p.ld_ss * 4);
                    }
                }
#pragma unroll
                for (int qq = 0; qq < QH; ++qq) {
                    const f32x4 zv = *reinterpret_cast<const f32x4*>(wl + (4 * (h + qq) + er) * ERS + ec * 16);
                    if (has_pre) st4(zv, rpa, vp, 4 * (h + qq) * (int)p.ld_preact * 4);
                    f32x4 y;
#pragma unroll
                    for (int e = 0; e < 4; ++e) {
                        float t = fmaf(zv[e], A[e], B[e]);
                        if constexpr (PERROW) t = fmaf(t, s1[qq][e] + 1.f, s2[qq][e]);
                        y[e] = dsc_silu_fast(t);
                    }
                    if (has_res) y += rres[qq];
                    st4(y, ry, vy, 4 * (h + qq) * (int)p.ldy * 4);
                }
            }
            if (c2 == 0) { DSC_WAVE_STAMP_KERNEL(5) }
        }
    }
    DSC_WAVE_STAMP_END
}

template <bool GN, int RB, bool PERROW = false, int J = 8, bool GB = false>
int launch(const dsc_gemm_args* a, const uint16_t* planes_f, int ntok, hipStream_t s) {
    const int scenes = (a->m + ntok - 1) / ntok;
    const unsigned grid = (unsigned)(((scenes + WAVES - 1) / WAVES) * (a->n / (16 * J)));
    DSC_CLEAR_STALE_ERROR();
    hipLaunchKernelGGL((gemm_split_wave_kernel<GN, RB, PERROW, J, GB>), dim3(grid, (unsigned)a->batch), dim3(64 * WAVES), 0, s, *a, planes_f, ntok DSC_WAVE_STAMP_PASS);
    DSC_LAUNCH_CHECK();
    return 0;
}

}
```

include/diffuscene_hip.h:

```cpp
#ifndef DIFFUSCENE_HIP_H
#define DIFFUSCENE_HIP_H

#include <stdint.h>

#ifdef __cplusplus
extern "C" {
#endif

typedef void* dsc_stream_t;

#define DSC_EINVAL   (-1)
#define DSC_EALIGN   (-2)
#define DSC_ERANGE   (-3)

#define DSC_ACT_NONE 0
#define DSC_ACT_GELU 1
#define DSC_ACT_SILU 2
#define DSC_ACT_LEAKY01 3

#define DSC_SS_NONE      0
#define DSC_SS_PER_TOKEN 1
#define DSC_SS_PER_SCENE 2
#define DSC_SS_PER_SLOT  3
#define DSC_SS_BY_INDEX  4

#define DSC_HEADS    4
#define DSC_DIM_HEAD 32

int dsc_version(void);

typedef struct dsc_gemm_args {
    const float* a1; int64_t lda1; int32_t k1;
    const float* a2; int64_t lda2; int32_t k2;
    const float* w;  int64_t ldw;
    const float* bias;
    const float* residual; int64_t ldr;
    float* y; int64_t ldy;
    int32_t m, n;
    int32_t act_in;
    int32_t act_out;
    int32_t batch; int64_t sa1, sa2, sw, sbias, sres, sy;
    const float* gamma; const float* beta; float eps;
    int32_t tokens_per_scene;
    const float* scale_shift; int64_t ld_ss; int32_t ss_mode;
    float* preact; int64_t ld_preact;
    const int64_t* ss_index;
    const uint16_t* w_planes;
    const float* actgrad_x; int64_t ld_actgrad;
    int32_t ss_rows;
    int32_t w_planes_layout;
    const float* gnb_z; int64_t ld_gnb_z;
    float* gnb_dgamma; float* gnb_dbeta; float* gnb_dbias; int64_t gnb_pstride;
    float* gnb_dss; int64_t ld_gnb_dss;
    int32_t flags;
} dsc_gemm_args;
#define DSC_GEMM_ROW_INVARIANT 1
#define DSC_PLANES_ROWMAJOR 0
#define DSC_PLANES_FRAGMENT 1
#define DSC_PLANES_NONE (-100)

int dsc_gemm_f32(const dsc_gemm_args* args, dsc_stream_t stream);

int dsc_gemm_arithmetic(const dsc_gemm_args* args, int32_t gn);

#define DSC_TILE_GN_32       0
#define DSC_TILE_GN_80_W8    1
#define DSC_TILE_GN_80_W4    2
#define DSC_TILE_GN_48       3
#define DSC_TILE_GN_64       4
#define DSC_TILE_160x256     5
#define DSC_TILE_256x128     6
#define DSC_TILE_128x128     7
#define DSC_TILE_160x128_W4  8
#define DSC_TILE_64x256      9
#define DSC_TILE_WAVE_GN     10
#define DSC_TILE_WAVE_DENSE  11
#define DSC_TILE_WAVE_GN_64  12
int dsc_gemm_split_tile(const dsc_gemm_args* args, int32_t gn);

#define DSC_F32_TILE_160x256 0
#define DSC_F32_TILE_160x128 1
#define DSC_F32_TILE_128x128 2
#define DSC_F32_TILE_96x128  3
#define DSC_F32_TILE_64x64   4
int dsc_gemm_f32_tile(const dsc_gemm_args* args);

int dsc_gemm_planes_layout(const dsc_gemm_args* args, int32_t gn);

int dsc_get_split_wave(void);
int dsc_set_split_wave(int32_t mode);

int dsc_gemm_skinny(const dsc_gemm_args* args, int32_t gn);
int dsc_get_skinny(void);
int dsc_set_skinny(int32_t on);

int dsc_get_gemm_arithmetic(void);
int dsc_set_gemm_arithmetic(int32_t mode);

#define DSC_SPLIT_TRANSPOSE 1
#define DSC_SPLIT_FRAGMENT  2
typedef struct dsc_split_item { const float* w; int64_t ldw; int32_t rows, cols; uint16_t* planes; int32_t transpose; } dsc_split_item;
int dsc_split_bf16x3_f32(const dsc_split_item* items, int32_t count, dsc_stream_t stream);

int dsc_gemm_gn_silu_f32(const dsc_gemm_args* args, dsc_stream_t stream);

int dsc_gemm_splitk_f32(const dsc_gemm_args* a, int32_t splits, float* workspace, int64_t workspace_floats, dsc_stream_t stream);

int dsc_gemm_layernorm_f32(const dsc_gemm_args* a, dsc_stream_t stream);

int dsc_linear_smallk_f32(const float* x, int64_t ldx, int32_t k_in, const float* w, int64_t ldw,
                          const float* bias, float* y, int64_t ldy, int32_t m, int32_t n,
                          int32_t act_out, dsc_stream_t stream);
#define DSC_SMALLK_MAX 4
typedef struct dsc_smallk_item { const float* x; int64_t ldx; int32_t k_in; const float* w; int64_t ldw; const float* bias;
                                 float* y; int64_t ldy; } dsc_smallk_item;
int dsc_linear_smallk_grouped_f32(const dsc_smallk_item* items, int32_t count, int32_t m, int32_t n, int32_t act_out,
                                  dsc_stream_t stream);
typedef struct dsc_col_span { int32_t src_col, dst_col, width; } dsc_col_span;
int dsc_gather_columns_f32(float* dst, int64_t ldd, const float* src, int64_t lds, int32_t rows, const dsc_col_span* spans,
                           int32_t count, dsc_stream_t stream);

#define DSC_WS_MAX 64
typedef struct dsc_ws_item { const float* w; float* out; int32_t rows; int32_t cols; } dsc_ws_item;
int dsc_weight_standardize_f32(const dsc_ws_item* items, int32_t count, float eps, dsc_stream_t stream);

int dsc_layernorm_f32(const float* x, int64_t ldx, const float* g, const float* residual, int64_t ldr,
                      float* y, int64_t ldy, int32_t m, int32_t d, float eps, dsc_stream_t stream);

int dsc_linear_attention_f32(const float* q, int64_t ldq, const float* k, int64_t ldk,
                             const float* v, int64_t ldv, float* out, int64_t ldo,
                             int32_t scenes, int32_t nq, int32_t nk, float scale, dsc_stream_t stream);

int dsc_attention_f32(const float* q, int64_t ldq, const float* k, int64_t ldk,
                      const float* v, int64_t ldv, float* out, int64_t ldo,
                      int32_t scenes, int32_t n, float scale, dsc_stream_t stream);

int dsc_time_embedding_f32(const int64_t* t, int32_t b, int32_t dim, const float* table, int32_t table_rows,
                           const float* freq, float* out, dsc_stream_t stream);

int dsc_activation_f32(const float* x, float* y, int64_t count, int32_t act, dsc_stream_t stream);


int64_t dsc_device_error_count(int32_t reset);

int dsc_q_sample_f32(const float* x0, const float* noise, const int64_t* t,
                     const float* sqrt_ac, const float* sqrt_1mac,
                     float* x_t, float* v_out, int32_t b, int64_t inner, int32_t num_timesteps, dsc_stream_t stream);

#define DSC_MEAN_EPS 0
#define DSC_MEAN_X0  1
#define DSC_MEAN_V   2
int dsc_p_sample_f32(const float* x_t, const float* model_out, const float* noise, const int64_t* t,
                     const float* ca, const float* cb, const float* coef1, const float* coef2,
                     const float* sigma, float* out, float* x0_out ,
                     int32_t mean_type, int32_t clip, int32_t b, int64_t inner, int32_t num_timesteps,
                     dsc_stream_t stream);

int dsc_add_scalar_i64(int64_t* t, int32_t count, int64_t delta, dsc_stream_t stream);

int dsc_ddim_step_f32(const float* x_t, const float* model_out, const float* noise, const int64_t* step,
                      const int64_t* times, const int64_t* times_next, const float* sqrt_alpha_next,
                      const float* c_noise, const float* sigma, const float* ca, const float* cb,
                      const float* sqrt_recip_ac, const float* sqrt_recipm1_ac, float* out, float* x0_out,
                      int32_t mean_type, int32_t b, int64_t inner, int32_t num_steps, int32_t num_timesteps,
                      dsc_stream_t stream);

int dsc_ddim_advance_i64(int64_t* step, const int64_t* times, int64_t* t, int32_t count, int32_t num_steps,
                         dsc_stream_t stream);

int dsc_postfilter_compact_f32(const float* samples, int32_t b, int32_t n, int32_t c, int32_t empty_col, int32_t mode,
                               int32_t keep_empty, float* packed, int32_t* counts, dsc_stream_t stream);

int dsc_complete_overwrite_f32(float* x, const float* partial, const float* noise, const int64_t* t,
                               const float* sqrt_ac, const float* sqrt_1mac,
                               int32_t b, int32_t n, int32_t p, int32_t c, int32_t num_timesteps, dsc_stream_t stream);

int dsc_complete_overwrite_ragged_f32(float* x, const float* partial, const float* noise, const int64_t* counts,
                                      const int64_t* t, const float* sqrt_ac, const float* sqrt_1mac,
                                      int32_t b, int32_t n, int32_t pmax, int32_t c, int32_t num_timesteps, dsc_stream_t stream);

int dsc_p_sample_inpaint_f32(const float* x_t, const float* model_out, const float* noise, const float* partial,
                             const float* noise_p, const int64_t* counts, const int64_t* t, const float* ca, const float* cb,
                             const float* coef1, const float* coef2, const float* sigma, const float* sqrt_ac,
                             const float* sqrt_1mac, float* out, int32_t mean_type, int32_t clip,
                             int32_t b, int32_t n, int32_t pmax, int32_t c, int32_t num_timesteps, dsc_stream_t stream);

int dsc_ddim_inpaint_step_f32(const float* x_t, const float* model_out, const float* noise, const float* partial,
                              const float* noise_p, const int64_t* counts, const int64_t* step, const int64_t* times,
                              const int64_t* times_next, const float* sqrt_alpha_next, const float* c_noise, const float* sigma,
                              const float* ca, const float* cb, const float* sqrt_recip_ac, const float* sqrt_recipm1_ac,
                              const float* sqrt_ac, const float* sqrt_1mac, float* out, int32_t mean_type,
                              int32_t b, int32_t n, int32_t pmax, int32_t c, int32_t num_steps, int32_t num_timesteps,
                              dsc_stream_t stream);

int dsc_masked_overwrite_f32(float* x, const float* known, const float* noise, const uint8_t* mask, const int64_t* t,
                             const float* sqrt_ac, const float* sqrt_1mac, int32_t b, int64_t inner, int32_t num_timesteps,
                             dsc_stream_t stream);

int dsc_p_sample_masked_f32(const float* x_t, const float* model_out, const float* noise, const float* known,
                            const float* noise_k, const uint8_t* mask, const int64_t* t, const float* ca, const float* cb,
                            const float* coef1, const float* coef2, const float* sigma, const float* sqrt_ac,
                            const float* sqrt_1mac, float* out, int32_t mean_type, int32_t clip, int32_t b, int64_t inner,
                            int32_t num_timesteps, dsc_stream_t stream);

int dsc_ddim_masked_step_f32(const float* x_t, const float* model_out, const float* noise, const float* known,
                             const float* noise_k, const uint8_t* mask, const int64_t* step, const int64_t* times,
                             const int64_t* times_next, const float* sqrt_alpha_next, const float* c_noise, const float* sigma,
                             const float* ca, const float* cb, const float* sqrt_recip_ac, const float* sqrt_recipm1_ac,
                             const float* sqrt_ac, const float* sqrt_1mac, float* out, int32_t mean_type,
                             int32_t b, int64_t inner, int32_t num_steps, int32_t num_timesteps, dsc_stream_t stream);

int dsc_cfg_combine_f32(const float* model_out, const float* scale, float* out, int32_t b, int64_t inner, dsc_stream_t stream);

int dsc_p_sample_cfg_f32(const float* x_t, const float* model_out, const float* scale, const float* noise, const int64_t* t,
                         const float* ca, const float* cb, const float* coef1, const float* coef2, const float* sigma,
                         float* out, float* x_dup , float* x0_out , int32_t mean_type,
                         int32_t clip, int32_t b, int64_t inner, int32_t num_timesteps, dsc_stream_t stream);

int dsc_ddim_cfg_step_f32(const float* x_t, const float* model_out, const float* scale, const float* noise, const int64_t* step,
                          const int64_t* times, const int64_t* times_next, const float* sqrt_alpha_next, const float* c_noise,
                          const float* sigma, const float* ca, const float* cb, const float* sqrt_recip_ac,
                          const float* sqrt_recipm1_ac, float* out, float* x_dup , float* x0_out ,
                          int32_t mean_type, int32_t b, int64_t inner, int32_t num_steps, int32_t num_timesteps,
                          dsc_stream_t stream);

int dsc_scene_gate_f32(const float* x, const uint8_t* keep, float* y, int32_t b, int64_t inner, dsc_stream_t stream);

int dsc_scene_randn_f32(float* out, const int64_t* seeds, const int64_t* draw, int64_t stream, int64_t b, int64_t per_scene,
                        dsc_stream_t hip_stream);
int dsc_scene_philox_u32(uint32_t* out, const int64_t* seeds, const int64_t* draw, int64_t stream, int64_t b, int64_t per_scene,
                         dsc_stream_t hip_stream);


int dsc_gemm_tn_f32(const float* a1, int64_t lda1, int32_t k1, const float* a2, int64_t lda2, int32_t k2,
                    const float* dy, int64_t ldd, float* out, int64_t ldo, float* dbias ,
                    int32_t m, int32_t n, int32_t kvalid, float* workspace, int64_t workspace_floats, dsc_stream_t stream);
int64_t dsc_gemm_tn_workspace_floats(int32_t m, int32_t n, int32_t k);

typedef struct dsc_tn_group {
    const float* a1; int64_t lda1; int32_t k1;
    const float* a2; int64_t lda2; int32_t k2;
    const float* dy; int64_t ldd;
    float* out; int64_t ldo;
    float* dbias;
    int32_t m, n, kvalid;
    int32_t tile0;
    int64_t ws_offset;
    int32_t tile0s;
} dsc_tn_group;
int dsc_gemm_tn_grouped_f32(const dsc_tn_group* groups_dev, int32_t count, int32_t total_tiles, int32_t splits,
                            float* workspace, int64_t workspace_floats, int64_t workspace_needed, dsc_stream_t stream);
int dsc_gemm_tn_grouped_split_f32(const dsc_tn_group* groups_dev, int32_t count, int32_t total_tiles, const int32_t* block_map_dev,
                                  int32_t blocks, int32_t splits, float* workspace, int64_t workspace_floats, int64_t workspace_needed,
                                  int32_t tile_k, dsc_stream_t stream);

int dsc_set_tn_split_form(int32_t form);
int dsc_get_tn_split_form(void);

int dsc_colsum_f32(const float* x, int64_t ldx, int32_t m, int32_t n, float* out, float* workspace,
                   int64_t workspace_floats, dsc_stream_t stream);

typedef struct dsc_colsum_item { const float* x; int64_t ldx; int32_t m, n; float* out; } dsc_colsum_item;
int dsc_colsum_grouped_f32(const dsc_colsum_item* items_dev, int32_t count, int32_t max_n, dsc_stream_t stream);

int dsc_gn_silu_bwd_f32(const float* z, int64_t ldz, const float* dy, int64_t ldy, const float* gamma,
                        const float* beta, const float* scale_shift, int64_t ld_ss, int32_t ss_mode,
                        float* dz, int64_t lddz, float* dgamma_p, float* dbeta_p, float* dbias_p, int64_t partial_stride,
                        float* dss, int64_t ld_dss, int32_t scenes, int32_t tokens_per_scene, int32_t channels,
                        float eps, dsc_stream_t stream);

typedef struct dsc_ws_bwd_item { const float* w; const float* dw_std; float* dw; int32_t rows; int32_t cols; } dsc_ws_bwd_item;
int dsc_weight_standardize_bwd_f32(const dsc_ws_bwd_item* items, int32_t count, float eps, dsc_stream_t stream);

int dsc_layernorm_bwd_f32(const float* x, int64_t ldx, const float* g, const float* dy, int64_t ldy, float* dx,
                          int64_t lddx, const float* addend, int64_t ldadd, float* dg_partial, int32_t partial_rows, int32_t m,
                          int32_t d, float eps, dsc_stream_t stream);

int dsc_linear_attention_bwd_f32(const float* q, int64_t ldq, const float* k, int64_t ldk, const float* v, int64_t ldv,
                                 const float* dout, int64_t ldo, float* dq, int64_t lddq, float* dk, int64_t lddk,
                                 float* dv, int64_t lddv, int32_t scenes, int32_t nq, int32_t nk, float scale,
                                 dsc_stream_t stream);

int dsc_attention_bwd_f32(const float* q, int64_t ldq, const float* k, int64_t ldk, const float* v, int64_t ldv,
                          const float* dout, int64_t ldo, float* dq, int64_t lddq, float* dk, int64_t lddk,
                          float* dv, int64_t lddv, int32_t scenes, int32_t n, float scale, dsc_stream_t stream);

int dsc_ddpm_loss_f32(const float* target, const float* out, const float* x_t, const int64_t* t,
                      const float* loss_weight, const float* ca, const float* cb, const float* alphas_cumprod,
                      const float* bounds, float* losses, float* parts, float* dout, int32_t b, int32_t n, int32_t c,
                      int32_t translation_dim, int32_t size_dim, int32_t bbox_dim, int32_t class_dim,
                      int32_t objectness_dim, int32_t objfeat_dim, int32_t loss_separate, int32_t loss_iou,
                      int32_t mean_type, float grad_scale, int32_t num_timesteps, dsc_stream_t stream);

int dsc_copy2d_f32(float* dst, int64_t ldd, const float* src, int64_t lds, int32_t rows, int32_t cols, dsc_stream_t stream);
int dsc_add2d_f32(float* dst, int64_t ldd, const float* src, int64_t lds, int32_t rows, int32_t cols, dsc_stream_t stream);

int dsc_activation_bwd_f32(const float* x, const float* dy, float* dx, int64_t count, int32_t act, dsc_stream_t stream);

int dsc_transpose_f32(const float* in, int64_t ldi, float* out, int64_t ldo, int32_t rows, int32_t cols,
                      dsc_stream_t stream);
int dsc_transpose_batched_f32(const dsc_ws_item* items, int32_t count, dsc_stream_t stream);

int dsc_retrieve_nearest_f32(const float* query_feats, const int32_t* query_labels, const double* query_sizes,
                             const float* db_feats, const int32_t* db_labels, const double* db_sizes,
                             int32_t n_query, int32_t n_db, int32_t feat_dim, int32_t* out_index, float* out_dist,
                             dsc_stream_t stream);

#define DSC_STATS_MAX_OBJECTS 160
#define DSC_STATS_ONE_WAVE_MAX 32

int dsc_box_bounds_f32(const float* translations, const float* sizes, const float* angles, const int32_t* counts,
                       int32_t batch, int32_t nmax, float* bounds, dsc_stream_t stream);

int dsc_scene_stats_f32(const float* bounds, const float* class_scores, const int32_t* model_ids, const int32_t* counts,
                        int32_t batch, int32_t nmax, int32_t num_classes, int32_t block_threads,
                        int32_t* num_intersecting, int32_t* num_symmetry, double* iou_sum, double* overlap_sum,
                        double* volume_sum, int32_t* class_counts, float* pair_iou, dsc_stream_t stream);

int dsc_encode_scene_batch_f32(const int64_t* offsets, const float* class_labels, const float* translations,
                               const float* sizes, const float* angles, const float* objfeats, int32_t n_cls_in,
                               int32_t feat_dim, const int64_t* scene, const int32_t* order, const double* rot,
                               const double* jitter, int32_t permute_objfeats, const double* bounds, float* out,
                               int64_t ld_out, int64_t* length, int32_t b, int32_t n, dsc_stream_t stream);

int dsc_chamfer3d_forward_f32(const float* xyz1, const float* xyz2, float* dist1, float* dist2, int32_t* idx1,
                              int32_t* idx2, int32_t b, int32_t n, int32_t m, dsc_stream_t stream);
int dsc_chamfer3d_backward_f32(const float* xyz1, const float* xyz2, const float* graddist1, const float* graddist2,
                               const int32_t* idx1, const int32_t* idx2, float* gradxyz1, float* gradxyz2, int32_t b,
                               int32_t n, int32_t m, dsc_stream_t stream);

typedef struct dsc_optim_chunk {
    float* param;
    const float* grad;
    float* exp_avg;
    float* exp_avg_sq;
    int64_t count;
} dsc_optim_chunk;

int dsc_grad_sumsq_f32(const dsc_optim_chunk* chunks, int32_t nchunks, double* partial, dsc_stream_t stream);
int dsc_clip_coef_f32(const double* partial, int32_t nchunks, float max_norm, float* total_norm, float* clip_coef,
                      dsc_stream_t stream);
int dsc_adam_step_f32(const dsc_optim_chunk* chunks, int32_t nchunks, float step_size, float beta1, float beta2,
                      float bias_correction2_sqrt, float eps, float weight_decay, const float* grad_scale,
                      dsc_stream_t stream);
int dsc_knn16_f32(const float* x, int64_t ldx, int32_t dim, const float* gram, const float* sqnorm, int32_t clouds, int32_t n,
                  int32_t* idx, dsc_stream_t stream);
int dsc_rowsq_f32(const float* x, int64_t ldx, int32_t dim, int64_t rows, float* out, dsc_stream_t stream);
int dsc_knn_cov_f32(const float* xyz, int64_t ldx, const int32_t* idx, int32_t clouds, int32_t n, float* out, int64_t ldo,
                    dsc_stream_t stream);
int dsc_gather_max_f32(const float* x, int64_t ldx, const int32_t* idx, int32_t clouds, int32_t n, int32_t ch, float* out,
                       int64_t ldo, uint8_t* arg, dsc_stream_t stream);
int dsc_gather_max_bwd_f32(const float* dy, int64_t ldy, const int32_t* idx, const uint8_t* arg, int32_t clouds, int32_t n,
                           int32_t ch, float* dx_zeroed, int64_t lddx, dsc_stream_t stream);
int64_t dsc_bn_workspace_floats(int64_t rows, int32_t ch);
int dsc_batchnorm_fwd_f32(const float* x, int64_t ldx, const float* gamma, const float* beta, int64_t rows, int32_t ch, float eps,
                          float momentum, int32_t relu, float* mean, float* rstd, float* running_mean, float* running_var,
                          float* xhat, float* y, float* workspace, int64_t workspace_floats, dsc_stream_t stream);
int dsc_batchnorm_eval_f32(const float* x, int64_t ldx, const float* gamma, const float* beta, const float* mean,
                           const float* rstd, int64_t rows, int32_t ch, int32_t relu, float* y, dsc_stream_t stream);
int dsc_batchnorm_bwd_f32(const float* dy, const float* xhat, const float* y, const float* gamma, const float* rstd, int64_t rows,
                          int32_t ch, int32_t relu, float* dx, float* dgamma, float* dbeta, float* workspace,
                          int64_t workspace_floats, dsc_stream_t stream);
int dsc_rowmax_f32(const float* x, int64_t ldx, int32_t clouds, int32_t n, int32_t ch, float* out, int32_t* arg,
                   dsc_stream_t stream);
int dsc_rowmax_bwd_f32(const float* dy, const int32_t* arg, int32_t clouds, int32_t n, int32_t ch, float* dx, dsc_stream_t stream);
int dsc_point_affine_f32(const float* x, int64_t ldx, int32_t x_per_cloud, const float* wp, int64_t ldw, const float* t,
                         int32_t clouds, int32_t n, int32_t ch, int32_t d, float* y, dsc_stream_t stream);
int dsc_point_affine_bwd_f32(const float* dy, const float* x, int64_t ldx, int32_t x_per_cloud, const float* wp, int64_t ldw,
                             int32_t clouds, int32_t n, int32_t ch, int32_t d, float* dx, int64_t lddx, float* dwp, int64_t lddw,
                             float* dt, float* workspace, int64_t workspace_floats, dsc_stream_t stream);

#ifdef __cplusplus
}
#endif
#endif
```

Baseline: 63.58 steps/s.

## Add two-waves-per-SIMD 80x64 wave GEMM variant with single-buffered LDS

Adds a PAIR template form of the split-bf16 wave GEMM kernel. It uses 64-channel tiles, launch bounds allowing two blocks per CU, a rotating two-slot register look-ahead, and an XCD-aware block order. It also halves each wave's LDS image to one stage for all variants and splits the transposed epilogue into row groups that fit that smaller image. The new width is chosen through a DSC_WAVE_PAIR switch, but the default rule returns false, so only the LDS and epilogue restructuring reach the default path. A new DSC_WAVE=2 mode forces wave tiles regardless of fill.

```diff
diff --git a/__graft_entry__.py b/__graft_entry__.py
--- a/__graft_entry__.py
+++ b/__graft_entry__.py
@@ -47,8 +47,7 @@
 
 def build(force=False):
     hipcc = _hipcc()
-    headers = [os.path.join(CSRC, "dsc_common.h"), os.path.join(CSRC, "gemm_core.h"), os.path.join(CSRC, "gemm_tn_split.h"),
-               os.path.join(ROOT, "include", "diffuscene_hip.h")]
+    headers = sorted(os.path.join(CSRC, h) for h in os.listdir(CSRC) if h.endswith(".h")) + [os.path.join(ROOT, "include", "diffuscene_hip.h")]
     objs = []
     for src, extra in SOURCES:
         s = os.path.join(CSRC, src)
diff --git a/diffuscene_amd/_lib.py b/diffuscene_amd/_lib.py
--- a/diffuscene_amd/_lib.py
+++ b/diffuscene_amd/_lib.py
@@ -106,6 +106,9 @@
     "dsc_gemm_planes_layout": (C.c_int, [C.POINTER(GemmArgs), C.c_int32]),
     "dsc_get_split_wave": (C.c_int, []),
     "dsc_set_split_wave": (C.c_int, [C.c_int32]),
+    "dsc_get_wave_pair": (C.c_int, []),
+    "dsc_set_wave_pair": (C.c_int, [C.c_int32]),
+    "dsc_gemm_wave_width": (C.c_int, [C.POINTER(GemmArgs), C.c_int32]),
     "dsc_gemm_skinny": (C.c_int, [C.POINTER(GemmArgs), C.c_int32]),
     "dsc_get_skinny": (C.c_int, []),
     "dsc_set_skinny": (C.c_int, [C.c_int32]),
@@ -254,7 +257,9 @@
     if lib.dsc_get_tn_split_form() < 0:
         raise ValueError("DSC_TN_FORM=%r: must be '2' (default), '1' or '0'" % os.environ.get("DSC_TN_FORM"))
     if lib.dsc_get_split_wave() < 0:
-        raise ValueError("DSC_WAVE=%r: must be '1' / 'auto' (default) or '0'" % os.environ.get("DSC_WAVE"))
+        raise ValueError("DSC_WAVE=%r: must be '1' / 'auto' (default), '0' or '2'" % os.environ.get("DSC_WAVE"))
+    if lib.dsc_get_wave_pair() < 0:
+        raise ValueError("DSC_WAVE_PAIR=%r: must be '1' (default), '0' or '2'" % os.environ.get("DSC_WAVE_PAIR"))
     _lib = lib
     return lib
 
@@ -267,12 +272,22 @@
     lib = load()
     if lib.dsc_get_gemm_arithmetic() != 1:
         return 0
-    return (2 if lib.dsc_get_split_wave() == 1 else 1) + 10 * lib.dsc_get_tn_split_form()
+    return (2 if lib.dsc_get_split_wave() >= 1 else 1) + 10 * lib.dsc_get_tn_split_form()
 
 
 def set_split_wave(on):
     prev = load().dsc_get_split_wave() == 1
     check(load().dsc_set_split_wave(1 if on else 0), "dsc_set_split_wave")
+    return prev
+
+
+def set_wave_switches(wave=None, pair=None):
+    lib = load()
+    prev = (lib.dsc_get_split_wave(), lib.dsc_get_wave_pair())
+    if wave is not None:
+        check(lib.dsc_set_split_wave(int(wave)), "dsc_set_split_wave")
+    if pair is not None:
+        check(lib.dsc_set_wave_pair(int(pair)), "dsc_set_wave_pair")
     return prev
 
 
diff --git a/diffuscene_amd/csrc/gemm_split.hip b/diffuscene_amd/csrc/gemm_split.hip
--- a/diffuscene_amd/csrc/gemm_split.hip
+++ b/diffuscene_amd/csrc/gemm_split.hip
@@ -448,20 +448,40 @@
     int m = g_split_wave.load(std::memory_order_relaxed);
     if (m == -1000) {
         const char* e = getenv("DSC_WAVE");
-        m = (!e || !e[0] || !strcmp(e, "1") || !strcmp(e, "auto")) ? 1 : !strcmp(e, "0") ? 0 : DSC_EINVAL;
+        m = (!e || !e[0] || !strcmp(e, "1") || !strcmp(e, "auto")) ? 1 : !strcmp(e, "0") ? 0 : !strcmp(e, "2") ? 2 : DSC_EINVAL;
         g_split_wave.store(m, std::memory_order_relaxed);
     }
     return m;
 }
 
 extern "C" int dsc_set_split_wave(int32_t mode) {
-    if (mode != 0 && mode != 1) return DSC_EINVAL;
+    if (mode < 0 || mode > 2) return DSC_EINVAL;
     g_split_wave.store(mode, std::memory_order_relaxed);
     return 0;
 }
 
+static std::atomic<int> g_wave_pair{-1000};
+
+extern "C" int dsc_get_wave_pair(void) {
+    int m = g_wave_pair.load(std::memory_order_relaxed);
+    if (m == -1000) {
+        const char* e = getenv("DSC_WAVE_PAIR");
+        m = (!e || !e[0] || !strcmp(e, "1")) ? 1 : !strcmp(e, "0") ? 0 : !strcmp(e, "2") ? 2 : DSC_EINVAL;
+        g_wave_pair.store(m, std::memory_order_relaxed);
+    }
+    return m;
+}
+
+extern "C" int dsc_set_wave_pair(int32_t mode) {
+    if (mode < 0 || mode > 2) return DSC_EINVAL;
+    g_wave_pair.store(mode, std::memory_order_relaxed);
+    return 0;
+}
+
 static int select_wave(const dsc_gemm_args* a, bool gn) {
-    if (dsc_get_split_wave() != 1) return -1;
+    const int wmode = dsc_get_split_wave();
+    if (wmode < 1) return -1;
+    const bool any_fill = wmode == 2;
     const int K = a->k1 + a->k2;
     if ((a->n % 128) || (a->k1 % 64) || (a->k2 % 64) || K < 256) return -1;
     if (a->batch != 1 && (gn || a->sw != (int64_t)a->n * K || a->ldw != K || (a->sy & 3) || (a->sres & 3) || (a->sbias & 3))) return -1;
@@ -484,7 +504,7 @@
         if (a->gnb_dss && (!dsc_aligned16(a->gnb_dss) || (a->ld_gnb_dss & 3))) return -1;
         waves = (long)(a->m / N) * (a->n / 128);
         const long r = (waves + 1023) / 1024;
-        return waves * 5 >= r * 1024 * 4 ? T_WAVE_DENSE : -1;
+        return (any_fill || waves * 5 >= r * 1024 * 4) ? T_WAVE_DENSE : -1;
     }
     if (gn) {
         const int N = a->tokens_per_scene;
@@ -496,12 +516,27 @@
         waves = (long)((a->m + 79) / 80) * (a->n / 128) * a->batch;
     }
     const long rounds = (waves + 1023) / 1024;
-    if (waves * 5 >= rounds * 1024 * 4) return gn ? T_WAVE_GN : T_WAVE_DENSE;
+    if (any_fill || waves * 5 >= rounds * 1024 * 4) return gn ? T_WAVE_GN : T_WAVE_DENSE;
     if (gn && a->tokens_per_scene > 64) {
         const long w4 = 2 * waves, r4 = (w4 + 1023) / 1024;
         if (r4 == 1 && w4 * 5 >= 1024 * 4) return T_WAVE_GN_64;
     }
     return -1;
+}
+
+static bool wave_pair_rule(const dsc_gemm_args* a, bool gn) {
+    (void)a; (void)gn;
+    return false;
+}
+
+static int select_wave_width(const dsc_gemm_args* a, bool gn, int tile) {
+    if (tile == T_WAVE_GN_64) return 64;
+    if (tile != T_WAVE_GN && tile != T_WAVE_DENSE) return 0;
+    const int mode = dsc_get_wave_pair();
+    if (mode < 1 || a->gnb_z) return 128;
+    if (gn && (a->tokens_per_scene <= 64 || a->tokens_per_scene > 80)) return 128;
+    if (mode == 2) return 64;
+    return wave_pair_rule(a, gn) ? 64 : 128;
 }
 
 static int select_block_tile(const dsc_gemm_args* a, bool gn);
@@ -553,7 +588,7 @@
 
 int dsc_gemm_try_split(const dsc_gemm_args* a, bool gn, hipStream_t s) {
     using namespace dsc_split;
-    if (dsc_get_gemm_arithmetic() < 0 || dsc_get_split_wave() < 0) return DSC_EINVAL;
+    if (dsc_get_gemm_arithmetic() < 0 || dsc_get_split_wave() < 0 || dsc_get_wave_pair() < 0) return DSC_EINVAL;
     const int N = a->tokens_per_scene;
     const int tile = select_tile(a, gn);
     if (tile < 0) return DSC_SPLIT_NOT_TAKEN;
@@ -572,6 +607,7 @@
         case T_64x256: return launch<false, 2, 4, 2>(a, 32, s);
         case T_WAVE_DENSE:
             if (a->gnb_z) return dsc_wave::launch<false, 5, false, 8, true>(a, a->w_planes, N, s);
+            if (select_wave_width(a, gn, tile) == 64) return dsc_wave::launch<false, 5, false, 4, false, true>(a, a->w_planes, 80, s);
             return dsc_wave::launch<false, 5>(a, a->w_planes, 80, s);
         case T_WAVE_GN_64:
             return (a->ss_mode == DSC_SS_PER_TOKEN || a->ss_mode == DSC_SS_PER_SLOT) ? dsc_wave::launch<true, 5, true, 4>(a, a->w_planes, N, s)
@@ -579,6 +615,8 @@
         case T_WAVE_GN: {
             const bool perrow = a->ss_mode == DSC_SS_PER_TOKEN || a->ss_mode == DSC_SS_PER_SLOT;
             const int rb = (N + 15) / 16;
+            if (select_wave_width(a, gn, tile) == 64)
+                return perrow ? dsc_wave::launch<true, 5, true, 4, false, true>(a, a->w_planes, N, s) : dsc_wave::launch<true, 5, false, 4, false, true>(a, a->w_planes, N, s);
             if (perrow) {
                 return rb == 5 ? dsc_wave::launch<true, 5, true>(a, a->w_planes, N, s) : rb == 4 ? dsc_wave::launch<true, 4, true>(a, a->w_planes, N, s)
                      : rb == 3 ? dsc_wave::launch<true, 3, true>(a, a->w_planes, N, s) : dsc_wave::launch<true, 2, true>(a, a->w_planes, N, s);
@@ -598,6 +636,12 @@
 extern "C" int dsc_gemm_split_tile(const dsc_gemm_args* a, int32_t gn) {
     if (!a || a->m <= 0 || a->n <= 0 || a->k1 <= 0) return DSC_EINVAL;
     return select_tile(a, gn != 0);
+}
+
+extern "C" int dsc_gemm_wave_width(const dsc_gemm_args* a, int32_t gn) {
+    if (!a || a->m <= 0 || a->n <= 0 || a->k1 <= 0) return DSC_EINVAL;
+    if (dsc_get_wave_pair() < 0) return DSC_EINVAL;
+    return select_wave_width(a, gn != 0, select_tile(a, gn != 0));
 }
 
 extern "C" int dsc_gemm_planes_layout(const dsc_gemm_args* a, int32_t gn) {
diff --git a/diffuscene_amd/csrc/gemm_split_wave.h b/diffuscene_amd/csrc/gemm_split_wave.h
--- a/diffuscene_amd/csrc/gemm_split_wave.h
+++ b/diffuscene_amd/csrc/gemm_split_wave.h
@@ -2,6 +2,9 @@
 #include "dsc_common.h"
 #include <utility>
 
+#ifndef DSC_WAVE_STORE_AUX
+#define DSC_WAVE_STORE_AUX 16
+#endif
 #ifndef DSC_WAVE_STAMP_ARGS
 #define DSC_WAVE_STAMP_ARGS
 #define DSC_WAVE_STAMP_PASS
@@ -47,12 +50,13 @@
 }
 
 template <int RB>
-constexpr int wave_smem_bytes() { return WAVES * 2 * 3 * (16 * RB) * 64; }
-
-template <bool GN, int RB, bool PERROW = false, int J = 8, bool GB = false>
-__global__ __launch_bounds__(64 * WAVES, 1) void gemm_split_wave_kernel(const dsc_gemm_args p, const uint16_t* const planes_f, const int ntok DSC_WAVE_STAMP_ARGS) {
+constexpr int wave_smem_bytes() { return WAVES * 3 * (16 * RB) * 64; }
+
+template <bool GN, int RB, bool PERROW = false, int J = 8, bool GB = false, bool PAIR = false>
+__global__ __launch_bounds__(64 * WAVES, PAIR ? 2 : 1) void gemm_split_wave_kernel(const dsc_gemm_args p, const uint16_t* const planes_f, const int ntok DSC_WAVE_STAMP_ARGS) {
     static_assert(J == 8 || J == 4, "wave tile: 128 or 64 channels");
     static_assert(!GB || (!GN && J == 8), "the GroupNorm-backward epilogue rides on the dense 80 x 128 form");
+    static_assert(!PAIR || (J == 4 && RB == 5 && 2 * wave_smem_bytes<RB>() <= 160 * 1024), "two waves per SIMD: 80 x 64 tiles, two blocks' LDS images per CU");
     constexpr int NWF = 3 * J;
     constexpr int CW = 16 * J;
     constexpr int ROWS = 16 * RB, XP = ROWS * 64, STAGE = 3 * XP;
@@ -68,8 +72,13 @@
     int sg, ch;
     if ((sgs & 7) == 0) {
         const int xcd = bid & 7, idx = bid >> 3;
-        sg = xcd * (sgs >> 3) + idx / chunks;
-        ch = idx % chunks;
+        if constexpr (PAIR) {
+            sg = xcd * (sgs >> 3) + idx % (sgs >> 3);
+            ch = idx / (sgs >> 3);
+        } else {
+            sg = xcd * (sgs >> 3) + idx / chunks;
+            ch = idx % chunks;
+        }
     } else {
         sg = bid / chunks;
         ch = bid % chunks;
@@ -103,7 +112,7 @@
     const int ildso = r16 * 64 + ((q4 ^ ((r16 >> 1) & 3)) << 4);
     const int xoff = l15 * 64 + ((g ^ ((l15 >> 1) & 3)) << 4);
     const int wvo = lane * 16;
-    char* const wl = smem + wave * (2 * STAGE);
+    char* const wl = smem + wave * STAGE;
 
     f32x4 acc[RB][J];
 #pragma unroll
@@ -114,27 +123,29 @@
         for (int i = 0; i < RB; ++i) acc[i][j] = b4;
     }
 
-    f32x4 ld[RB][2];
+    constexpr int NLD = PAIR ? 2 : RB;
+    f32x4 ld[NLD][2];
     bf16x8 wf[2][J][3], xf[2][3];
     const int lda2e = p.a2 ? (int)p.lda2 : (int)p.lda1, kshift = p.a2 ? p.k1 : 0;
     const int tvo2e = p.a2 ? tvo2 : tvo1;
-    auto load_tok = [&](int kt, int u, auto segc) {
+    auto load_rows = [&](f32x4 (&dst)[2], int kt, int u, auto segc) {
 #if defined(__HIP_DEVICE_COMPILE__)
         constexpr int SEG = decltype(segc)::value;
         const int k0 = kt * BK;
         if constexpr (SEG == 0) {
             const int so = (u * 16 * (int)p.lda1 + k0) * 4;
-            ld[u][0] = __builtin_bit_cast(f32x4, __builtin_amdgcn_raw_buffer_load_b128(r1, tvo1, so, 0));
-            ld[u][1] = __builtin_bit_cast(f32x4, __builtin_amdgcn_raw_buffer_load_b128(r1, tvo1 + 16, so, 0));
+            dst[0] = __builtin_bit_cast(f32x4, __builtin_amdgcn_raw_buffer_load_b128(r1, tvo1, so, 0));
+            dst[1] = __builtin_bit_cast(f32x4, __builtin_amdgcn_raw_buffer_load_b128(r1, tvo1 + 16, so, 0));
         } else {
             const int so = (u * 16 * lda2e + k0 - kshift) * 4;
-            ld[u][0] = __builtin_bit_cast(f32x4, __builtin_amdgcn_raw_buffer_load_b128(r2, tvo2e, so, 0));
-            ld[u][1] = __builtin_bit_cast(f32x4, __builtin_amdgcn_raw_buffer_load_b128(r2, tvo2e + 16, so, 0));
+            dst[0] = __builtin_bit_cast(f32x4, __builtin_amdgcn_raw_buffer_load_b128(r2, tvo2e, so, 0));
+            dst[1] = __builtin_bit_cast(f32x4, __builtin_amdgcn_raw_buffer_load_b128(r2, tvo2e + 16, so, 0));
         }
 #else
-        (void)kt; (void)u;
+        (void)dst; (void)kt; (void)u;
 #endif
     };
+    auto load_tok = [&](int kt, int u, auto segc) { load_rows(ld[PAIR ? 0 : u], kt, u, segc); };
     auto load_w = [&](int kt, int j, int pl) -> bf16x8 {
 #if defined(__HIP_DEVICE_COMPILE__)
         return __builtin_bit_cast(bf16x8, __builtin_amdgcn_raw_buffer_load_b128(rw, wvo, pl * plane_bytes + ((nb0 + j) * KT + kt) * 1024, 0));
@@ -146,9 +157,12 @@
     constexpr int NMMA = 6 * J;
 
     auto tile = [&](const int kt, auto curc, auto segc) {
-        constexpr int CUR = decltype(curc)::value, NXT = CUR ^ 1;
-        char* const cur = wl + CUR * STAGE;
-        char* const nxt = wl + NXT * STAGE;
+        constexpr int CUR = decltype(curc)::value, NXT = CUR ^ 1, SEGC = decltype(segc)::value;
+        static_assert(PAIR || SEGC < 2, "mixed look-ahead: the PAIR form only");
+        using seg1c = std::integral_constant<int, SEGC == 1 ? 1 : 0>;
+        using seg2c = std::integral_constant<int, SEGC == 0 ? 0 : 1>;
+        char* const cur = wl;
+        char* const nxt = wl;
         const int kn1 = min(kt + 1, KT - 1), kn2 = min(kt + 2, KT - 1);
         constexpr int X0 = CUR ? (RB & 1) : 0;
         DSC_WAVE_STAMP_TILE(0)
@@ -161,7 +175,8 @@
             static_assert(S3 <= NMMA, "one MFMA per filler slot");
             unsigned su1[4], su2[4], su3[4];
             float sr0[4], sr1[4], st0[4], st1[4];
-            auto xin = [&](int q, int h) -> float { return q < 2 ? ld[i][0][2 * q + h] : ld[i][1][2 * q - 4 + h]; };
+            constexpr int LS = PAIR ? (CUR + i + 1) & 1 : i;
+            auto xin = [&](int q, int h) -> float { return q < 2 ? ld[LS][0][2 * q + h] : ld[LS][1][2 * q - 4 + h]; };
             auto split_op = [&](auto nc) {
                 constexpr int n = decltype(nc)::value;
                 constexpr int q = 2 * (n / 22) + (n & 1), o = (n % 22) >> 1;
@@ -194,7 +209,9 @@
                                                                                               : u32x4{su3[0], su3[1], su3[2], su3[3]};
                     *reinterpret_cast<u32x4*>(d0 + pl * XP) = v;
                 } else if constexpr (k == S2) {
-                    load_tok(kn2, i, segc);
+                    if constexpr (!PAIR) load_tok(kn2, i, seg2c{});
+                    else if constexpr (i + 2 < RB) load_rows(ld[LS], kn1, i + 2, seg1c{});
+                    else load_rows(ld[LS], kn2, i + 2 - RB, seg2c{});
                 }
             };
             auto product = [&](auto pc) {
@@ -216,19 +233,25 @@
     };
 
     using std::integral_constant;
-#pragma unroll
-    for (int u = 0; u < RB; ++u) load_tok(0, u, integral_constant<int, 0>{});
+    f32x4 ld0[PAIR ? RB : 1][2];
+#pragma unroll
+    for (int u = 0; u < RB; ++u) {
+        if constexpr (PAIR) load_rows(ld0[PAIR ? u : 0], 0, u, integral_constant<int, 0>{});
+        else load_tok(0, u, integral_constant<int, 0>{});
+    }
 #pragma unroll
     for (int w = 0; w < NWF; ++w) wf[0][w / 3][w % 3] = load_w(0, w / 3, w % 3);
 #pragma unroll
     for (int u = 0; u < RB; ++u) {
         bf16x8 a, b, c;
-        split8(ld[u][0], ld[u][1], a, b, c);
+        if constexpr (PAIR) split8(ld0[PAIR ? u : 0][0], ld0[PAIR ? u : 0][1], a, b, c);
+        else split8(ld[PAIR ? 0 : u][0], ld[PAIR ? 0 : u][1], a, b, c);
         char* d0 = wl + u * 1024 + ildso;
         *reinterpret_cast<bf16x8*>(d0) = a;
         *reinterpret_cast<bf16x8*>(d0 + XP) = b;
         *reinterpret_cast<bf16x8*>(d0 + 2 * XP) = c;
-        load_tok(1, u, integral_constant<int, 0>{});
+        if constexpr (!PAIR) load_tok(1, u, integral_constant<int, 0>{});
+        else if (u < 2) load_rows(ld[(u + 1) & 1], 1, u, integral_constant<int, 0>{});
     }
 #pragma unroll
     for (int pl = 0; pl < 3; ++pl) xf[0][pl] = *reinterpret_cast<const bf16x8*>(wl + pl * XP + xoff);
@@ -258,6 +281,11 @@
             }
         }
     }
+    if constexpr (PAIR) {
+        tile(kt, integral_constant<int, 0>{}, integral_constant<int, 2>{});
+        tile(kt + 1, integral_constant<int, 1>{}, integral_constant<int, 1>{});
+        kt += 2;
+    }
     for (; kt < KT; kt += 2) {
         tile(kt, integral_constant<int, 0>{}, integral_constant<int, 1>{});
         tile(kt + 1, integral_constant<int, 1>{}, integral_constant<int, 1>{});
@@ -265,7 +293,8 @@
 
     DSC_WAVE_STAMP_KERNEL(2)
     constexpr int ERS = 64 * 4 + 16;
-    static_assert(ROWS * ERS <= 2 * STAGE, "the transposed cell fits the wave's LDS image");
+    constexpr int EG = STAGE / (16 * ERS) < RB ? STAGE / (16 * ERS) : RB, NG = (RB + EG - 1) / EG;
+    static_assert(EG >= 1 && EG * 16 * ERS <= STAGE, "a row group of the transposed cell fits the wave's LDS image");
     const int er = lane >> 4, ec = lane & 15;
 #if defined(__HIP_DEVICE_COMPILE__)
     auto row_rsrc = [&](const float* base, int64_t ld, int rows, int cols) {
@@ -276,20 +305,24 @@
     const __amdgpu_buffer_rsrc_t rpa = row_rsrc(p.preact ? p.preact + (int64_t)z * p.sy + (int64_t)row0 * p.ld_preact : p.y, p.ld_preact, p.preact ? rows_here : 0, p.n);
     auto ld4 = [&](const __amdgpu_buffer_rsrc_t& r, int voff, int soff) { return __builtin_bit_cast(f32x4, __builtin_amdgcn_raw_buffer_load_b128(r, voff, soff, 0)); };
     auto st4 = [&](const f32x4 v, const __amdgpu_buffer_rsrc_t& r, int voff, int soff) { __builtin_amdgcn_raw_buffer_store_b128(__builtin_bit_cast(u32x4, v), r, voff, soff, 0); };
+    auto st4y = [&](const f32x4 v, const __amdgpu_buffer_rsrc_t& r, int voff, int soff) { __builtin_amdgcn_raw_buffer_store_b128(__builtin_bit_cast(u32x4, v), r, voff, soff, DSC_WAVE_STORE_AUX); };
 #else
     const int ry = 0, rr = 0, rpa = 0;
     auto ld4 = [&](int, int, int) { return f32x4{}; };
     auto st4 = [&](const f32x4, int, int, int) {};
+    auto st4y = st4;
 #endif
     const bool has_res = p.residual != nullptr, has_pre = p.preact != nullptr;
-    auto to_lds = [&](const int c2) {
-#pragma unroll
-        for (int i = 0; i < RB; ++i)
-#pragma unroll
-            for (int j = 0; j < 4; ++j) *reinterpret_cast<f32x4*>(wl + (i * 16 + l15) * ERS + (j * 16 + 4 * g) * 4) = acc[i][4 * c2 + j];
+    auto to_lds = [&](auto c2c, auto gic) {
+        constexpr int c2 = decltype(c2c)::value, gi = decltype(gic)::value;
+        constexpr int I0 = gi * EG, I1 = (gi + 1) * EG < RB ? (gi + 1) * EG : RB;
+#pragma unroll
+        for (int i = I0; i < I1; ++i)
+#pragma unroll
+            for (int j = 0; j < 4; ++j) *reinterpret_cast<f32x4*>(wl + ((i - I0) * 16 + l15) * ERS + (j * 16 + 4 * g) * 4) = acc[i][4 * c2 + j];
     };
-    constexpr int NQ = ROWS / 4, QH = NQ % 10 == 0 ? 10 : NQ % 8 == 0 ? 8 : NQ % 6 == 0 ? 6 : 4;
-    static_assert(NQ % QH == 0, "row groups per pass");
+    auto from_lds = [&](const int q, const int gi) { return *reinterpret_cast<const f32x4*>(wl + (4 * q + er - 16 * EG * gi) * ERS + ec * 16); };
+    constexpr int NQ = ROWS / 4, QH = 4 * EG;
     if constexpr (GB) {
         const float inv_cnt = 1.f / (float)(ntok * 64);
         const bool per_scene = p.ss_mode == DSC_SS_PER_SCENE && p.scale_shift;
@@ -312,11 +345,15 @@
                 s1 = *reinterpret_cast<const f32x4*>(ssr) + 1.f;
                 sh = *reinterpret_cast<const f32x4*>(ssr + p.n);
             }
-            to_lds(c2);
+            dsc_static_for<NG>([&](auto gic) {
+                constexpr int gi = decltype(gic)::value;
+                to_lds(c2c, gic);
+#pragma unroll
+                for (int q = gi * QH; q < (gi * QH + QH < NQ ? gi * QH + QH : NQ); ++q) dv[q] = from_lds(q, gi);
+            });
             float s = 0.f;
 #pragma unroll
             for (int q = 0; q < NQ; ++q) {
-                dv[q] = *reinterpret_cast<const f32x4*>(wl + (4 * q + er) * ERS + ec * 16);
                 const bool ok = 4 * q + er < rows_here;
                 if (!ok) dv[q] = f32x4{0.f, 0.f, 0.f, 0.f};
                 s += ok ? (zv[q][0] + zv[q][1]) + (zv[q][2] + zv[q][3]) : 0.f;
@@ -356,7 +393,7 @@
                 f32x4 dzv;
 #pragma unroll
                 for (int e = 0; e < 4; ++e) { dzv[e] = rs * (dv[q][e] - m1 - zv[q][e] * m2); Gz[e] += ok ? dzv[e] : 0.f; }
-                st4(dzv, ry, vy, 4 * q * (int)p.ldy * 4);
+                st4y(dzv, ry, vy, 4 * q * (int)p.ldy * 4);
             }
             auto fold = [&](f32x4 v) {
 #pragma unroll
@@ -382,25 +419,25 @@
 #else
         const int rg = 0;
 #endif
-        auto cell = [&](auto c2c, auto modec, auto actc) {
+        auto cell = [&](auto c2c, auto modec, auto actc) __attribute__((always_inline)) {
             constexpr int c2 = decltype(c2c)::value, MODE = decltype(modec)::value, ACT = decltype(actc)::value;
             const int cc = (col0 + 64 * c2 + 4 * ec) * 4;
             const int vy = er * (int)p.ldy * 4 + cc, vr = er * (int)p.ldr * 4 + cc, vp = er * (int)p.ld_preact * 4 + cc, vg = er * (int)p.ld_actgrad * 4 + cc;
-            to_lds(c2);
-#pragma unroll 1
-            for (int h = 0; h < NQ; h += QH) {
-                f32x4 rres[QH], gx[QH];
+            dsc_static_for<NG>([&](auto gic) {
+                constexpr int gi = decltype(gic)::value, h = gi * QH, QN = h + QH < NQ ? QH : NQ - h;
+                to_lds(c2c, gic);
+                f32x4 rres[QN], gx[QN];
                 if (has_res) {
 #pragma unroll
-                    for (int qq = 0; qq < QH; ++qq) rres[qq] = ld4(rr, vr, 4 * (h + qq) * (int)p.ldr * 4);
+                    for (int qq = 0; qq < QN; ++qq) rres[qq] = ld4(rr, vr, 4 * (h + qq) * (int)p.ldr * 4);
                 }
                 if constexpr (MODE == 2) {
 #pragma unroll
-                    for (int qq = 0; qq < QH; ++qq) gx[qq] = ld4(rg, vg, 4 * (h + qq) * (int)p.ld_actgrad * 4);
-                }
-#pragma unroll
-                for (int qq = 0; qq < QH; ++qq) {
-                    f32x4 y = *reinterpret_cast<const f32x4*>(wl + (4 * (h + qq) + er) * ERS + ec * 16);
+                    for (int qq = 0; qq < QN; ++qq) gx[qq] = ld4(rg, vg, 4 * (h + qq) * (int)p.ld_actgrad * 4);
+                }
+#pragma unroll
+                for (int qq = 0; qq < QN; ++qq) {
+                    f32x4 y = from_lds(h + qq, gi);
                     if (has_pre) st4(y, rpa, vp, 4 * (h + qq) * (int)p.ld_preact * 4);
 #pragma unroll
                     for (int e = 0; e < 4; ++e) {
@@ -408,11 +445,11 @@
                         if constexpr (MODE == 2) y[e] *= dsc_act_grad(gx[qq][e], ACT);
                     }
                     if (has_res) y += rres[qq];
-                    st4(y, ry, vy, 4 * (h + qq) * (int)p.ldy * 4);
-                }
-            }
+                    st4y(y, ry, vy, 4 * (h + qq) * (int)p.ldy * 4);
+                }
+            });
         };
-        auto cells = [&](auto modec, auto actc) {
+        auto cells = [&](auto modec, auto actc) __attribute__((always_inline)) {
             cell(std::integral_constant<int, 0>{}, modec, actc);
             if constexpr (J == 8) cell(std::integral_constant<int, 1>{}, modec, actc);
         };
@@ -438,11 +475,11 @@
 #endif
         const float inv_cnt = 1.f / (float)(ntok * 64);
         const bool vlast = (RB - 1) * 16 + l15 < rows_here;
-#pragma unroll
-        for (int c2 = 0; c2 < J / 4; ++c2) {
+        dsc_static_for<J / 4>([&](auto c2c) {
+            constexpr int c2 = decltype(c2c)::value;
             const int ch = col0 + 64 * c2 + 4 * ec;
             const f32x4 ga = ep_ga[c2], be = ep_be[c2], sc = ep_sc[c2], sh = ep_sh[c2];
-            to_lds(c2);
+            to_lds(c2c, std::integral_constant<int, 0>{});
             float s0 = 0.f;
 #pragma unroll
             for (int i = 0; i < RB; ++i)
@@ -475,23 +512,24 @@
             const int cc = ch * 4;
             const int vy = er * (int)p.ldy * 4 + cc, vr = er * (int)p.ldr * 4 + cc, vp = er * (int)p.ld_preact * 4 + cc, vs = er * (int)p.ld_ss * 4 + cc;
             if (c2 == 0) { DSC_WAVE_STAMP_KERNEL(4) }
-#pragma unroll
-            for (int h = 0; h < NQ; h += QH) {
-                f32x4 rres[QH], s1[QH], s2[QH];
+            dsc_static_for<NG>([&](auto gic) {
+                constexpr int gi = decltype(gic)::value, h = gi * QH, QN = h + QH < NQ ? QH : NQ - h;
+                if constexpr (gi > 0) to_lds(c2c, gic);
+                f32x4 rres[QN], s1[QN], s2[QN];
                 if (has_res) {
 #pragma unroll
-                    for (int qq = 0; qq < QH; ++qq) rres[qq] = ld4(rr, vr, 4 * (h + qq) * (int)p.ldr * 4);
+                    for (int qq = 0; qq < QN; ++qq) rres[qq] = ld4(rr, vr, 4 * (h + qq) * (int)p.ldr * 4);
                 }
                 if constexpr (PERROW) {
 #pragma unroll
-                    for (int qq = 0; qq < QH; ++qq) {
+                    for (int qq = 0; qq < QN; ++qq) {
                         s1[qq] = ld4(rs, vs, 4 * (h + qq) * (int)p.ld_ss * 4);
                         s2[qq] = ld4(rs, vs + p.n * 4, 4 * (h + qq) * (int)p.ld_ss * 4);
                     }
                 }
 #pragma unroll
-                for (int qq = 0; qq < QH; ++qq) {
-                    const f32x4 zv = *reinterpret_cast<const f32x4*>(wl + (4 * (h + qq) + er) * ERS + ec * 16);
+                for (int qq = 0; qq < QN; ++qq) {
+                    const f32x4 zv = from_lds(h + qq, gi);
                     if (has_pre) st4(zv, rpa, vp, 4 * (h + qq) * (int)p.ld_preact * 4);
                     f32x4 y;
 #pragma unroll
@@ -501,21 +539,21 @@
                         y[e] = dsc_silu_fast(t);
                     }
                     if (has_res) y += rres[qq];
-                    st4(y, ry, vy, 4 * (h + qq) * (int)p.ldy * 4);
-                }
-            }
+                    st4y(y, ry, vy, 4 * (h + qq) * (int)p.ldy * 4);
+                }
+            });
             if (c2 == 0) { DSC_WAVE_STAMP_KERNEL(5) }
-        }
+        });
     }
     DSC_WAVE_STAMP_END
 }
 
-template <bool GN, int RB, bool PERROW = false, int J = 8, bool GB = false>
+template <bool GN, int RB, bool PERROW = false, int J = 8, bool GB = false, bool PAIR = false>
 int launch(const dsc_gemm_args* a, const uint16_t* planes_f, int ntok, hipStream_t s) {
     const int scenes = (a->m + ntok - 1) / ntok;
     const unsigned grid = (unsigned)(((scenes + WAVES - 1) / WAVES) * (a->n / (16 * J)));
     DSC_CLEAR_STALE_ERROR();
-    hipLaunchKernelGGL((gemm_split_wave_kernel<GN, RB, PERROW, J, GB>), dim3(grid, (unsigned)a->batch), dim3(64 * WAVES), 0, s, *a, planes_f, ntok DSC_WAVE_STAMP_PASS);
+    hipLaunchKernelGGL((gemm_split_wave_kernel<GN, RB, PERROW, J, GB, PAIR>), dim3(grid, (unsigned)a->batch), dim3(64 * WAVES), 0, s, *a, planes_f, ntok DSC_WAVE_STAMP_PASS);
     DSC_LAUNCH_CHECK();
     return 0;
 }
diff --git a/include/diffuscene_hip.h b/include/diffuscene_hip.h
--- a/include/diffuscene_hip.h
+++ b/include/diffuscene_hip.h
@@ -89,6 +89,10 @@
 
 int dsc_get_split_wave(void);
 int dsc_set_split_wave(int32_t mode);
+
+int dsc_get_wave_pair(void);
+int dsc_set_wave_pair(int32_t mode);
+int dsc_gemm_wave_width(const dsc_gemm_args* args, int32_t gn);
 
 int dsc_gemm_skinny(const dsc_gemm_args* args, int32_t gn);
 int dsc_get_skinny(void);
```

Result: no change. 63.66 steps/s, median of 2 (+0.1%).
